# panuelosj/polystokes

Measured on AMD Instinct MI355X. Metric: Stokes-solve wall ms/step (assembly+PCG) on 256^3 grid; CG iters/sec, lower is better.
Workload: dtype f64; 1 GPU; synthetic lid-driven cavity 256x256x256, reduced tiles (tile=16, pad=2), jacobi-PCG, tol 1e-3; parallelism=1 GPU

## Files before the change

polystokes_amd/__init__.py:

```python
import ctypes as C
import os
import subprocess

import numpy as np

from . import _abi
from ._abi import (FieldsIn, FieldsOut, Params, Scene, Stats, default_params)

_HERE = os.path.dirname(os.path.abspath(__file__))
LIB_PATH = os.environ.get("PS_LIB") or os.path.join(_HERE, "libpolystokes_hip.so")
_lib = None

EXPORTED_SYMBOLS = [
    "ps_abi_version", "ps_reduced_dof", "ps_context_create", "ps_context_destroy", "ps_last_error", "ps_params_default",
    "ps_upload_fields", "ps_step_device", "ps_setup_device", "ps_solve_device", "ps_download_fields",
    "polystokes_step", "ps_apply_operator", "ps_apply_preconditioner", "ps_query_array", "ps_read_array",
    "ps_export_component_matrices", "ps_export_matrices", "ps_export_stats", "ps_bench_kernel", "ps_memory_stats", "ps_set_interrupt", "ps_solve_exported_system",
    "ps_set_slab", "ps_set_brick", "ps_comm_unique_id", "ps_comm_init_rccl", "ps_comm_selftest", "ps_comm_init_tcp", "ps_dist_stats",
    "ps_group_create", "ps_group_destroy", "ps_group_rank", "ps_group_step",
    "ps_set_warm_start", "ps_download_solution_fields", "ps_upload_density_field", "ps_set_surface_tension",
    "ps_set_solid_boundary", "ps_set_rheology", "ps_set_solve_precision",
    "ps_upload_fields_device", "ps_upload_density_field_device", "ps_download_fields_device", "ps_download_solution_fields_device",
    "ps_step_device_fields", "ps_set_velocity_extrapolation",
    "ps_upload_surface_fields", "ps_upload_surface_fields_device",
# ... 39 lines not shown
        L.ps_apply_preconditioner.argtypes = [C.c_void_p, C.c_void_p, C.c_void_p]
        L.ps_apply_preconditioner.restype = C.c_int32
        L.ps_query_array.argtypes = [C.c_void_p, C.c_char_p, C.POINTER(C.c_int32)]
        L.ps_query_array.restype = C.c_int64
        L.ps_read_array.argtypes = [C.c_void_p, C.c_char_p, C.c_void_p, C.c_int64]
        L.ps_read_array.restype = C.c_int32
        L.ps_export_component_matrices.argtypes = [C.c_void_p, C.c_char_p]
        L.ps_export_component_matrices.restype = C.c_int32
        L.ps_export_matrices.argtypes = [C.c_void_p, C.c_char_p]
        L.ps_export_matrices.restype = C.c_int32
        L.ps_export_stats.argtypes = [C.c_void_p, C.POINTER(Stats), C.c_char_p]
        L.ps_export_stats.restype = C.c_int32
        L.ps_bench_kernel.argtypes = [C.c_void_p, C.c_char_p, C.c_int32, C.POINTER(C.c_double), C.POINTER(C.c_double)]
        L.ps_bench_kernel.restype = C.c_int32
        L.ps_memory_stats.argtypes = [C.c_void_p, C.POINTER(C.c_int64)]
        L.ps_memory_stats.restype = C.c_int32
        L.ps_solve_exported_system.argtypes = [C.c_void_p, C.c_char_p, C.POINTER(Params), C.c_double, C.c_void_p, C.c_int64, C.POINTER(Stats)]
        L.ps_solve_exported_system.restype = C.c_int32
        L.ps_set_interrupt.argtypes = [C.c_void_p, C.c_void_p, C.c_void_p]
        L.ps_set_interrupt.restype = C.c_int32
        L.ps_set_slab.argtypes = [C.c_void_p, C.POINTER(_abi.SlabStruct)]
        L.ps_set_slab.restype = C.c_int32
        L.ps_set_brick.argtypes = [C.c_void_p, C.POINTER(_abi.BrickStruct)]
        L.ps_set_brick.restype = C.c_int32
        L.ps_comm_unique_id.argtypes = [C.c_void_p]
        L.ps_comm_unique_id.restype = C.c_int32
        L.ps_comm_init_rccl.argtypes = [C.c_void_p, C.c_void_p, C.c_int32, C.c_int32]
        L.ps_comm_init_rccl.restype = C.c_int32
        L.ps_comm_init_tcp.argtypes = [C.c_void_p, C.c_int32, C.c_int32, C.c_char_p, C.c_int32]
        L.ps_comm_init_tcp.restype = C.c_int32
        L.ps_comm_selftest.argtypes = [C.c_void_p]
        L.ps_comm_selftest.restype = C.c_int32
        L.ps_dist_stats.argtypes = [C.c_void_p, C.POINTER(C.c_double)]
        L.ps_dist_stats.restype = C.c_int32
        L.ps_group_create.argtypes = [C.c_int32, C.c_int32]
        L.ps_group_create.restype = C.c_void_p
        L.ps_group_destroy.argtypes = [C.c_void_p]
        L.ps_group_rank.argtypes = [C.c_void_p, C.c_int32]
        L.ps_group_rank.restype = C.c_void_p
        L.ps_group_step.argtypes = [C.c_void_p, C.POINTER(Stats)]
        L.ps_group_step.restype = C.c_int32
        L.ps_set_warm_start.argtypes = [C.c_void_p, C.c_int32]
        L.ps_set_warm_start.restype = C.c_int32
        L.ps_download_solution_fields.argtypes = [C.c_void_p, C.POINTER(_abi.SolutionOut)]
        L.ps_download_solution_fields.restype = C.c_int32
        L.ps_upload_density_field.argtypes = [C.c_void_p, C.c_void_p]
        L.ps_upload_density_field.restype = C.c_int32
        L.ps_set_surface_tension.argtypes = [C.c_void_p, C.c_double]
        L.ps_set_surface_tension.restype = C.c_int32
        L.ps_set_solid_boundary.argtypes = [C.c_void_p, C.c_int32]
        L.ps_set_solid_boundary.restype = C.c_int32
        L.ps_set_rheology.argtypes = [C.c_void_p, C.POINTER(_abi.Rheology)]
        L.ps_set_rheology.restype = C.c_int32
        L.ps_set_solve_precision.argtypes = [C.c_void_p, C.c_int32]
        L.ps_set_solve_precision.restype = C.c_int32
        L.ps_set_velocity_extrapolation.argtypes = [C.c_void_p, C.c_int32]
        L.ps_set_velocity_extrapolation.restype = C.c_int32
        L.ps_upload_fields_device.argtypes = [C.c_void_p, C.POINTER(Params), C.POINTER(FieldsIn), C.c_int32, C.c_void_p]
        L.ps_upload_fields_device.restype = C.c_int32
        L.ps_upload_density_field_device.argtypes = [C.c_void_p, C.c_void_p, C.c_int32, C.c_void_p]
        L.ps_upload_density_field_device.restype = C.c_int32
        L.ps_download_fields_device.argtypes = [C.c_void_p, C.POINTER(FieldsOut), C.c_int32, C.c_void_p]
        L.ps_download_fields_device.restype = C.c_int32
        L.ps_download_solution_fields_device.argtypes = [C.c_void_p, C.POINTER(_abi.SolutionOut), C.c_int32, C.c_void_p]
        L.ps_download_solution_fields_device.restype = C.c_int32
        L.ps_step_device_fields.argtypes = [C.c_void_p, C.POINTER(Params), C.POINTER(FieldsIn), C.POINTER(FieldsOut), C.POINTER(Stats),
                                            C.c_int32, C.c_void_p]
        L.ps_step_device_fields.restype = C.c_int32
        L.ps_upload_surface_fields.argtypes = [C.c_void_p, C.POINTER(_abi.SurfaceFields)]
        L.ps_upload_surface_fields.restype = C.c_int32
        L.ps_upload_surface_fields_device.argtypes = [C.c_void_p, C.POINTER(_abi.SurfaceFields), C.c_int32, C.c_void_p]
        L.ps_upload_surface_fields_device.restype = C.c_int32
        _lib = L
    return _lib


def device_address(a):
    if a is None:
        return None
    if isinstance(a, int):
        return a
    if hasattr(a, "ptr"):
        return int(a.ptr)
    if hasattr(a, "data_ptr"):
        return int(a.data_ptr())
    if hasattr(a, "__cuda_array_interface__"):
        return int(a.__cuda_array_interface__["data"][0])
    raise TypeError(f"no device address in {type(a).__name__}")


def stream_handle(stream):
    if stream is None:
        return None
    return int(stream) if isinstance(stream, int) else int(stream.cuda_stream)


def to_layout(a, layout):
    a = np.asarray(a, dtype=np.float32)
    return np.ascontiguousarray(a if layout == _abi.LAYOUT_X_FASTEST else a.transpose(2, 1, 0))


def from_layout(flat, shape_zyx, layout):
    flat = np.asarray(flat).ravel()
    if layout == _abi.LAYOUT_X_FASTEST:
        return flat.reshape(shape_zyx)
    return np.ascontiguousarray(flat.reshape(shape_zyx[::-1]).transpose(2, 1, 0))


class DeviceScene:

    def __init__(self, scene, layout=_abi.LAYOUT_X_FASTEST, pad=0):
        from . import _hip
        put = lambda a: _hip.DeviceBuffer.from_numpy(to_layout(a, layout), pad)
        self.layout, self.host = layout, scene
        for k in ("nx", "ny", "nz", "dx", "dt", "density", "name", "surface_tension"):
            setattr(self, k, getattr(scene, k))
        self.vel = [put(a) for a in scene.vel]
        self.collisionvel = [put(a) for a in scene.collisionvel]
        self.surface, self.collision, self.viscosity = put(scene.surface), put(scene.collision), put(scene.viscosity)
        self.weights = None if scene.weights is None else [put(a) for a in scene.weights]
        self.density_field = None if scene.density_field is None else put(scene.density_field)
        opt = lambda name: None if getattr(scene, name, None) is None else put(getattr(scene, name))
        self.surface_sigma_field, self.surface_pressure_field = opt("surface_sigma_field"), opt("surface_pressure_field")


def device_scene(scene, layout=_abi.LAYOUT_X_FASTEST, pad=0):
    return DeviceScene(scene, layout, pad)


def fields_in_device(fields):
    fi = FieldsIn()
    fi.nx, fi.ny, fi.nz = fields.nx, fields.ny, fields.nz
    fi.dx, fi.dt = fields.dx, fields.dt
    fi.orig[0] = fi.orig[1] = fi.orig[2] = 0.0
    fi.density = fields.density
    cv = getattr(fields, "collisionvel", None)
    for a in range(3):
        fi.vel[a] = device_address(fields.vel[a])
        fi.collisionvel[a] = device_address(cv[a]) if cv is not None else None
    fi.surface, fi.collision, fi.viscosity = (device_address(fields.surface), device_address(fields.collision),
                                              device_address(fields.viscosity))
    w = getattr(fields, "weights", None)
    for i in range(14):
        fi.weights[i] = device_address(w[i]) if w is not None else None
    return fi


_DT = {(1, "i"): np.int8, (4, "i"): np.int32, (4, "f"): np.float32, (8, "f"): np.float64, (4, "u"): np.uint32}


def _kind(name):
    if name.endswith(("Labels", "Indices", ".col", ".ptr", "Region", "Perm", ".chunkInfo", ".chunkRep", ".code")) or name.startswith("faceRow"):
        return "i"
    if name in ("valuesCoded", "columns16", "diagonalsCoded", "fusedStep", "streamRuns", "rowPerLane", "chebInner32", "warmStartUsed", "densityField", "launchWalk",
                "surfaceTensionReducedFaces", "surfaceFields", "solidBoundary", "solidSlipEdges", "rheologyModel", "rheologyIterations",
                "solvePrecisionUsed", "solvePassIterations",
                "velocityExtrapolation", "extrapolationLayerX", "extrapolationLayerY", "extrapolationLayerZ", "extrapolationCounts"):
        return "i"
    if name in ("ownedX", "ownedY", "ownedZ"):
        return "f"
    if False:
        return "i"
    if name == "reducedRowFace":
        return "u"
    return "f"


def process_memory_stats():
    v = (C.c_int64 * 4)()
    lib().ps_memory_stats(None, v)
    return {"live_bytes": int(v[0]), "peak_bytes": int(v[1]), "contexts": int(v[3])}


def _has_surface_fields(scene):
    return getattr(scene, "surface_sigma_field", None) is not None or getattr(scene, "surface_pressure_field", None) is not None


class PolyStokesError(RuntimeError):
    pass


class Solver:

    def __init__(self, device=0, _handle=None):
        self.L = lib()
        self._owned = _handle is None
        h = self.L.ps_context_create(device) if _handle is None else _handle
        if not h:
            raise PolyStokesError(self.L.ps_last_error(None).decode())
        self.h = C.c_void_p(h)
        self.stats = Stats()
        self.scene = None

    def close(self):
        if getattr(self, "h", None):
            if self._owned:
                self.L.ps_context_destroy(self.h)
            self.h = None

    def set_interrupt(self, fn):
        if fn is None:
            self._cb = None
            self._check(self.L.ps_set_interrupt(self.h, None, None))
            return
        self._cb = C.CFUNCTYPE(C.c_int32, C.c_void_p)(lambda user: 1 if fn() else 0)
        self._check(self.L.ps_set_interrupt(self.h, C.cast(self._cb, C.c_void_p), None))

    def set_warm_start(self, mode):
        self._check(self.L.ps_set_warm_start(self.h, int(mode)))

    def set_surface_tension(self, sigma):
        return self._check(self.L.ps_set_surface_tension(self.h, float(sigma)), allow=(1, -2))

    def set_solid_boundary(self, mode):
        return self._check(self.L.ps_set_solid_boundary(self.h, int(mode)), allow=(1, -2))

    def set_rheology(self, model=_abi.RHEOLOGY_HERSCHEL_BULKLEY, flow_index=1.0, yield_stress=0.0, min_shear_rate=1e-3,
                     min_viscosity=1e-3, max_viscosity=1e6, passes=0):
        r = _abi.Rheology(int(model), int(passes), float(flow_index), float(yield_stress), float(min_shear_rate), float(min_viscosity),
                          float(max_viscosity))
        return self._check(self.L.ps_set_rheology(self.h, C.byref(r)), allow=(1, -2))

    def set_solve_precision(self, mode):
        return self._check(self.L.ps_set_solve_precision(self.h, int(mode)), allow=(1, -2))

    def set_velocity_extrapolation(self, layers):
        return self._check(self.L.ps_set_velocity_extrapolation(self.h, int(layers)), allow=(1, -2))

    def solution_fields(self):
        sh = _abi.grid_shapes(self.scene.nx, self.scene.ny, self.scene.nz)
        out = {name: np.empty(sh[grid], np.float32) for name, grid in _abi.SOLUTION_FIELDS}
        so = _abi.SolutionOut()
        so.pressure = out["pressure"].ctypes.data
        for a, name in enumerate(("txx", "tyy", "tzz")):
            so.tauDiag[a] = out[name].ctypes.data
        for a, name in enumerate(("tyz", "txz", "txy")):
            so.tauEdge[a] = out[name].ctypes.data
        self._check(self.L.ps_download_solution_fields(self.h, C.byref(so)))
        return out

    def set_slab(self, slab):
        st = _abi.SlabStruct(slab.rank, slab.world, slab.zLoOwned, slab.zHiOwned, slab.hasLower, slab.hasUpper, slab.z0)
        self._check(self.L.ps_set_slab(self.h, C.byref(st)))

    def set_brick(self, b):
        i3 = C.c_int32 * 3
        st = _abi.BrickStruct(b.rank, b.world, i3(*b.dims), i3(*b.lo), i3(*b.hi), i3(*b.hasLower), i3(*b.hasUpper), i3(*b.g0))
        self._check(self.L.ps_set_brick(self.h, C.byref(st)))

    def comm_selftest(self):
        self._check(self.L.ps_comm_selftest(self.h))

    def dist_stats(self):
        v = (C.c_double * 8)()
        self._check(self.L.ps_dist_stats(self.h, v))
        return {"halo_bytes_per_iter": v[0], "owned_dofs": v[1], "overlap": bool(v[2]),
                "exchange_ms_per_transport": (v[3] / v[4]) if v[4] else None, "exchange_samples": int(v[4]),
                "allreduce_ms": (v[5] / v[6]) if v[6] else None, "allreduce_samples": int(v[6]), "halo_label_changes": int(v[7])}

    def memory_stats(self):
        v = (C.c_int64 * 4)()
        self.L.ps_memory_stats(self.h, v)
        return {"live_bytes": int(v[0]), "peak_bytes": int(v[1]), "deferred_bytes": int(v[2]), "contexts": int(v[3])}

    def comm_init(self, uid_bytes, rank, world):
        buf = C.create_string_buffer(bytes(uid_bytes), 128)
        self._check(self.L.ps_comm_init_rccl(self.h, buf, rank, world))

    def comm_init_tcp(self, rank, world, host="127.0.0.1", base_port=29600):
        self._check(self.L.ps_comm_init_tcp(self.h, rank, world, host.encode(), base_port))

    def __del__(self):
        try:
            self.close()
        except Exception:
            pass

    def _check(self, rc, allow=(1,)):
        if rc == _abi.FAILED or rc not in allow:
            raise PolyStokesError(f"rc={rc}: {self.L.ps_last_error(self.h).decode()}")
        return rc

    def upload(self, scene, params):
        self.scene, self.params = scene, params
        fi = scene.fields_in()
        self._check(self.L.ps_upload_fields(self.h, C.byref(params), C.byref(fi)))
        self._scene_surface_tension(scene)
        if getattr(scene, "density_field", None) is not None:
            self._check(self.upload_density_field(scene.density_field))
        if _has_surface_fields(scene):
            self._check(self.upload_surface_fields(scene.surface_sigma_field, scene.surface_pressure_field))

    def _scene_surface_tension(self, scene):
        sigma = getattr(scene, "surface_tension", None)
        if sigma is not None:
            self._check(self.L.ps_set_surface_tension(self.h, float(sigma)))

    def upload_density_field(self, field):
        if field is None:
            return self._check(self.L.ps_upload_density_field(self.h, None), allow=(1, -2))
        sh = _abi.grid_shapes(self.scene.nx, self.scene.ny, self.scene.nz)["center"] if self.scene is not None else None
        f = np.ascontiguousarray(field, dtype=np.float32)
        if sh is not None and f.shape != sh:
            f = f.reshape(sh)
        self._density_keep = f
        return self._check(self.L.ps_upload_density_field(self.h, f.ctypes.data), allow=(1, -2))

# ... 284 lines not shown
```

polystokes_amd/csrc/ps_blocks.hip:

```cpp
#include "ps_context.hpp"
#include "ps_setup_util.hpp"

using namespace ps;

namespace {

constexpr int BS = SETUP_BS;

struct BlockArgs {
    Grid g;
    double invDx;
    const float* lw[7];
    const float* fw[7];
    const int32_t* lab[7];
    const int32_t* act[7];
    const int32_t* reg[7];
    const int32_t* sys[7];
    const int32_t* sysT[3];
    const int32_t* faceRow[3];
    const float* vel[3];
    const float* cvel[3];
    CellField visc;
    FaceDensity dens;
    int64_t nP, nA, faceOff[3];
// ... 378 lines not shown
        cnt[j] = n;
        if (slipEdge(A, ea, c)) atomicAdd(A.slipEdges, 1);
        return;
    }
    sortRows4(rows, vals);
    const int p0 = ptr[j];
#pragma unroll
    for (int k = 0; k < 4; ++k)
        if (k < n) { col[p0 + k] = rows[k]; if (val) val[p0 + k] = vals[k]; code[p0 + k] = encodeVal(A, vals[k]); }
    rhsPT[j] = rhs;
    const double vw = clampd((double)A.fw[4 + ea][c], 0.1, 1.0) * (double)A.lw[4 + ea][c];
    const float ox = ea == 0 ? 0.5f : 0.f, oy = ea == 1 ? 0.5f : 0.f, oz = ea == 2 ? 0.5f : 0.f;
    const double visc = (double)A.visc.sample(A.g, (float)q.x + ox, (float)q.y + oy, (float)q.z + oz);
    const double invVisc = clampd(1. / visc, 0., 1e10);
    uInv[t] = A.own.sample(4 + ea, q.x, q.y, q.z) ? 2. * invVisc * vw : 0.;
    if (uDiag) uDiag[t] = 0.5 * visc * clampd(1. / vw, 0., 1.e2);
}

BlockArgs makeArgs(ps_context* c) {
    BlockArgs A;
    A.g = c->g; A.invDx = c->invDx;
    for (int s = 0; s < 7; ++s) {
        A.lw[s] = c->liquidW[s].p; A.fw[s] = c->fluidW[s].p;
        A.lab[s] = c->labels[s].p; A.act[s] = c->activeIdx[s].p; A.reg[s] = c->reducedIdx[s].p; A.sys[s] = c->sysIdx[s].p;
    }
    for (int a = 0; a < 3; ++a) { A.faceRow[a] = c->faceRow[a].p; A.vel[a] = c->vel[a].p; A.cvel[a] = c->cvel[a].p; A.sysT[a] = c->sysIdxT[a].p; }
    A.visc = c->viscSource(); A.dens = c->densSource();
    A.nP = c->nPressures; A.nA = c->nActiveVs;
    A.faceOff[0] = 0; A.faceOff[1] = c->nFace[0]; A.faceOff[2] = c->nFace[0] + c->nFace[1];
    A.own = c->own();
    A.valScale = c->valScale;
    A.codeFail = c->counters.p + CTR_CODE_FAIL;
    A.regionOwned = (c->slabEnabled && c->regionCount > 0) ? c->regionOwned.p : nullptr;
    A.freeSlip = c->solidBoundaryUsed == PS_SOLID_FREE_SLIP ? 1 : 0;
    A.slipEdges = A.freeSlip ? c->slipEdges.p : nullptr;
    return A;
}

__global__ void k_chunk_len4(const int32_t* __restrict__ ptr, const int2* __restrict__ chunkRows, int nChunks, int32_t* __restrict__ len4, int32_t* __restrict__ maxLen) {
    const int ch = blockIdx.x * blockDim.x + threadIdx.x;
    if (ch > nChunks) return;
    int n = 0;
    if (ch < nChunks) { const int2 cr = chunkRows[ch]; n = ptr[cr.x + cr.y] - ptr[cr.x]; atomicMax(maxLen, n); }
    len4[ch] = (n + 3) & ~3;
}
__global__ void __launch_bounds__(BS) k_col16_build(const int32_t* __restrict__ ptr, const int32_t* __restrict__ col, const int8_t* __restrict__ code,
                                                    const int2* __restrict__ chunkRows, const int32_t* __restrict__ start4, uint16_t* __restrict__ col16,
                                                    int8_t* __restrict__ code4, int32_t* __restrict__ winBase, int4* __restrict__ chunkInfo,
                                                    uint8_t* __restrict__ len8, int32_t* __restrict__ fail, int32_t* __restrict__ chunkRep, int nChunks) {
    const int lane = threadIdx.x & 63;
    const int chunk = blockIdx.x * (BS / 64) + (int)(threadIdx.x >> 6);
    if (chunk >= nChunks) return;
    if (lane == 0) chunkRep[chunk] = chunk;
    const int2 cr = chunkRows[chunk];
    const int r0 = cr.x;
    const int p0 = ptr[r0], p1 = ptr[r0 + cr.y];
    const int q0 = start4[chunk], q1 = start4[chunk + 1];
    if (lane == 0) chunkInfo[chunk] = make_int4(q0, (p1 - p0) | (cr.y << 16), cr.x, cr.x);
    for (int i = lane; i < cr.y; i += 64) len8[r0 + i] = (uint8_t)(ptr[r0 + i + 1] - ptr[r0 + i]);
    constexpr int SL = 32;
    if (p1 - p0 > SL * 64) { if (lane == 0) *fail = 1; return; }
    int c[SL];
    unsigned open = 0u;
#pragma unroll
    for (int u = 0; u < SL; ++u) {
        const int i = lane + u * 64;
        const bool o = p0 + i < p1;
        c[u] = o ? col[p0 + i] : 0x7fffffff;
        if (o) open |= 1u << u;
        if (q0 + i < q1) { code4[q0 + i] = o ? code[p0 + i] : (int8_t)0; if (!o) col16[q0 + i] = 0; }
    }
    int used = 16;
    for (int w = 0; w < 16; ++w) {
        int m = 0x7fffffff;
#pragma unroll
        for (int u = 0; u < SL; ++u) if ((open >> u) & 1u) m = min(m, c[u]);
        for (int o = 32; o > 0; o >>= 1) m = min(m, __shfl_xor(m, o));
        const int base = m;
        if (base == 0x7fffffff) { used = w; break; }
        if (lane == 0) winBase[(int64_t)chunk * 16 + w] = base;
#pragma unroll
        for (int u = 0; u < SL; ++u)
            if (((open >> u) & 1u) && c[u] - base < 4096) {
                col16[q0 + lane + u * 64] = (uint16_t)((w << 12) | (c[u] - base));
                open &= ~(1u << u);
            }
    }
    if (lane == 0) for (int w = used; w < 16; ++w) winBase[(int64_t)chunk * 16 + w] = 0;
    if (open) *fail = 1;
}
__global__ void __launch_bounds__(64) k_chunk_hash(const int4* __restrict__ chunkInfo, const uint16_t* __restrict__ col16, const int8_t* __restrict__ code4,
                                                   const uint8_t* __restrict__ len8, unsigned long long* __restrict__ hash, int weak) {
    const int chunk = blockIdx.x;
    const int4 ci = chunkInfo[chunk];
    const int n4 = ((ci.y & 0xffff) + 3) & ~3, rows = (int)((unsigned)ci.y >> 16);
    unsigned long long h = 0;
    if (!weak)
    for (int i = threadIdx.x; i < n4; i += 64)
        h += mix64(((unsigned long long)i << 32) | ((unsigned long long)col16[ci.x + i] << 8) | (uint8_t)code4[ci.x + i]);
    if (!weak)
    for (int i = threadIdx.x; i < rows; i += 64) h += mix64(0x4000000000000000ull | ((unsigned long long)i << 32) | len8[ci.z + i]);
    for (int o = 32; o > 0; o >>= 1) h += __shfl_down(h, o, 64);
    if (threadIdx.x == 0) {
        h = mix64(h ^ (((unsigned long long)(unsigned)n4 << 32) | (unsigned)rows));
        hash[chunk] = h == HASH_EMPTY ? 0ull : h;
    }
}
__global__ void k_chunk_rep_insert(const unsigned long long* __restrict__ hash, int nChunks, unsigned long long* __restrict__ keys, int32_t* __restrict__ vals, unsigned mask) {
    const int chunk = blockIdx.x * blockDim.x + threadIdx.x;
    if (chunk >= nChunks) return;
    const unsigned long long h = hash[chunk];
    hashInsertMin(keys, vals, mask, (unsigned)(h >> 17) & mask, h, chunk);
}
__global__ void __launch_bounds__(64) k_chunk_share(const unsigned long long* __restrict__ hash, const unsigned long long* __restrict__ keys, const int32_t* __restrict__ vals,
                                                    unsigned mask, int4* __restrict__ chunkInfo, const uint16_t* __restrict__ col16, const int8_t* __restrict__ code4,
                                                    const uint8_t* __restrict__ len8, const uint8_t* __restrict__ rowCode, int codeRows,
                                                    unsigned long long* __restrict__ uniqueLen, int32_t* __restrict__ chunkRep) {
    const int chunk = blockIdx.x;
    const unsigned long long h = hash[chunk];
    unsigned slot = (unsigned)(h >> 17) & mask;
    while (keys[slot] != h) slot = (slot + 1) & mask;
    const int rep = vals[slot];
    const int4 ci = chunkInfo[chunk];
    const int n = ci.y & 0xffff, n4 = (n + 3) & ~3, rows = (int)((unsigned)ci.y >> 16);
    bool same = rep != chunk;
    if (same) {
        const int4 cr = chunkInfo[rep];
        same = cr.y == ci.y;
        if (same) {
            for (int i = threadIdx.x; i < n4; i += 64) same = same && col16[ci.x + i] == col16[cr.x + i] && code4[ci.x + i] == code4[cr.x + i];
            for (int i = threadIdx.x; i < rows; i += 64) {
                same = same && len8[ci.z + i] == len8[cr.z + i];
                if (rowCode) {
                    const bool a = ci.z + i < codeRows, b = cr.z + i < codeRows;
                    same = same && a == b && (!a || rowCode[ci.z + i] == rowCode[cr.z + i]);
                }
            }
        }
        same = __all(same) != 0;
        if (same && threadIdx.x == 0) { chunkInfo[chunk].x = cr.x; chunkInfo[chunk].w = cr.z; chunkRep[chunk] = rep; }
    }
    if (!same && threadIdx.x == 0) atomicAdd(uniqueLen, (unsigned long long)n4);
}
__global__ void __launch_bounds__(BS) k_val4_build(const int32_t* __restrict__ ptr, const double* __restrict__ val,
                                                   const int4* __restrict__ chunkInfo, double* __restrict__ val4) {
    const int chunk = blockIdx.x;
    const int4 ci = chunkInfo[chunk];
    const int p0 = ptr[ci.z], n = ci.y & 0xffff, q0 = ci.x;
    const int n4 = (n + 3) & ~3;
    for (int i = threadIdx.x; i < n4; i += BS) val4[q0 + i] = i < n ? val[p0 + i] : 0.;
}
__device__ inline int ellCodeWidth(int W) { return W > 4 ? 8 : (W > 0 ? 4 : 0); }
constexpr int32_t ELL_NULL_BASE = 0x1ffff000;
__global__ void __launch_bounds__(BS) k_ell_plan(const int4* __restrict__ chunkInfo, const uint8_t* __restrict__ len8, const int32_t* __restrict__ chunkRep,
                                                 int32_t* __restrict__ colLen, int32_t* __restrict__ codeLen, int32_t* __restrict__ wpack, int32_t* __restrict__ fail) {
    __shared__ int wmax[BS / 64];
    const int chunk = blockIdx.x;
    const int4 ci = chunkInfo[chunk];
    const int rows = (int)((unsigned)ci.y >> 16);
    int len = (int)threadIdx.x < rows ? (int)len8[ci.z + threadIdx.x] : 0;
    for (int o = 32; o > 0; o >>= 1) len = max(len, __shfl_down(len, o, 64));
    if ((threadIdx.x & 63) == 0) wmax[threadIdx.x >> 6] = len;
    __syncthreads();
    if (threadIdx.x == 0) {
        int cl = 0, vl = 0, wp = 0;
        for (int u = 0; u < BS / 64; ++u) {
            const int W = (wmax[u] + 1) & ~1;
            if (W > 8) *fail = 1;
            cl += 64 * W; vl += 64 * ellCodeWidth(W); wp |= (W & 15) << (4 * u);
        }
        const bool own = chunkRep[chunk] == chunk;
        colLen[chunk] = own ? cl : 0; codeLen[chunk] = own ? vl : 0; wpack[chunk] = wp;
    }
}
__global__ void __launch_bounds__(BS) k_ell_fill(const int4* __restrict__ chunkInfo, const uint8_t* __restrict__ len8, const int32_t* __restrict__ chunkRep,
                                                 const uint16_t* __restrict__ col16, const int8_t* __restrict__ code4, const int32_t* __restrict__ colBegin,
                                                 const int32_t* __restrict__ codeBegin, const int32_t* __restrict__ wpack, uint16_t* __restrict__ ecol,
                                                 int8_t* __restrict__ ecode, int4* __restrict__ echunk, int32_t* __restrict__ winBase) {
    const int chunk = blockIdx.x;
    const int rep = chunkRep[chunk];
    const bool nullOk = winBase[chunk * 16 + 15] == 0 || winBase[chunk * 16 + 15] == ELL_NULL_BASE;
    __syncthreads();
    if (nullOk && threadIdx.x == 0) winBase[chunk * 16 + 15] = ELL_NULL_BASE;
    const int4 ci = chunkInfo[chunk];
    const int rows = (int)((unsigned)ci.y >> 16);
    const int wp = wpack[chunk];
    if (threadIdx.x == 0) echunk[chunk] = make_int4(colBegin[rep], codeBegin[rep], ci.z, rows | (wp << 12));
    if (rep != chunk) return;
    const int len = (int)len8[ci.z + min((int)threadIdx.x, rows - 1)];
    int total;
    const int mine = (int)threadIdx.x < rows ? len : 0;
    const int e0 = blockExclusiveScan(mine, &total);
    __shared__ int lastE0;
    if ((int)threadIdx.x == rows - 1) lastE0 = e0;
    __syncthreads();
    const int eb = ci.x + ((int)threadIdx.x < rows ? e0 : lastE0);
    const int u = threadIdx.x >> 6, lane = threadIdx.x & 63;
    const int W = (wp >> (4 * u)) & 15, CW = ellCodeWidth(W);
    if (W == 0 || u * 64 >= rows) return;
    int pre = 0, preC = 0;
    for (int v = 0; v < u; ++v) { const int w = (wp >> (4 * v)) & 15; pre += w; preC += ellCodeWidth(w); }
    uint16_t* oc = ecol + (size_t)colBegin[chunk] + (size_t)64 * pre + (size_t)lane * W;
    int8_t* ov = ecode + (size_t)codeBegin[chunk] + (size_t)64 * preC + (size_t)lane * CW;
    uint16_t lastc = 0;
    for (int k = 0; k < W; ++k) {
        if (k < len) lastc = col16[eb + k];
        oc[k] = (k < len || !nullOk) ? lastc : (uint16_t)0xf000;
    }
    for (int k = 0; k < CW; ++k) ov[k] = k < len ? code4[eb + k] : (int8_t)0;
}
}
void ps_context::buildEll(ps::DevCSR& M) {
    M.ellok = false;
    static const bool off = envInt(PS_ENV("PS_NO_ELL"), 0) != 0 ||
                            envInt(PS_ENV("PS_PIPE_GRID"), 1) == 0;
    if (off || !M.col16ok || !M.packed || M.nChunks == 0 || (uint64_t)std::max(M.rows, M.cols) * 8 >= 0xffff8000ull) return;
    const int nChunks = M.nChunks;
    DevBuf<int32_t>& colBegin = scrEllCol; DevBuf<int32_t>& codeBegin = scrEllCode; DevBuf<int32_t>& wpack = scrEllW;
    colBegin.alloc((size_t)nChunks + 1); codeBegin.alloc((size_t)nChunks + 1); wpack.alloc((size_t)nChunks);
    HIP_CHECK(hipMemsetAsync(colBegin.p + nChunks, 0, sizeof(int32_t), stream));
    HIP_CHECK(hipMemsetAsync(codeBegin.p + nChunks, 0, sizeof(int32_t), stream));
    HIP_CHECK(hipMemsetAsync(counters.p + CTR_ELL_TOO_LONG, 0, sizeof(int32_t), stream));
    hipLaunchKernelGGL(k_ell_plan, dim3((unsigned)nChunks), dim3(BS), 0, stream, (const int4*)M.chunkInfo.p, (const uint8_t*)M.len8.p, (const int32_t*)M.chunkRep.p,
                       colBegin.p, codeBegin.p, wpack.p, counters.p + CTR_ELL_TOO_LONG);
    scanBlock.alloc((size_t)gridFor(nChunks + 1, PS_SCAN_TILE) + 16);
    (void)exclusiveScanI32(colBegin.p, nChunks + 1, CTR_ELL_COLS);
    (void)exclusiveScanI32(codeBegin.p, nChunks + 1, CTR_ELL_CODES);
    int32_t w[3];
    fetchCounters(CTR_ELL_TOO_LONG, 3, w);
    const int32_t tooLong = w[0];
    const int64_t totCol = w[1], totCode = w[2];
    if (totCol < 0 || totCode < 0 || (uint64_t)totCol * 2 >= 0xffffffffull || tooLong != 0) return;
    M.ellCols = totCol; M.ellCodes = totCode; M.ellUniqueCols = totCol;
    M.ecol.alloc((size_t)totCol + 64); M.ecode.alloc((size_t)totCode + 64); M.echunk.alloc((size_t)nChunks);
    hipLaunchKernelGGL(k_ell_fill, dim3((unsigned)nChunks), dim3(BS), 0, stream, (const int4*)M.chunkInfo.p, (const uint8_t*)M.len8.p, (const int32_t*)M.chunkRep.p,
                       (const uint16_t*)M.col16.p, (const int8_t*)M.code4.p, (const int32_t*)colBegin.p, (const int32_t*)codeBegin.p, (const int32_t*)wpack.p,
                       M.ecol.p, M.ecode.p, M.echunk.p, M.winBase.p);
    M.ellok = true;
    if (PS_ENV_VERBOSE()) std::fprintf(stderr, "[polystokes] row-per-lane stream: %d chunks, %lld column slots and %lld code bytes in the distinct runs (nnz %lld)\n",
                                           nChunks, (long long)totCol, (long long)totCode, (long long)M.nnz);
}
namespace {
__global__ void k_decode_values(const int8_t* __restrict__ code, double scale, int64_t n, double* __restrict__ val) {
    for (int64_t i = (int64_t)blockIdx.x * blockDim.x + threadIdx.x; i < n; i += (int64_t)gridDim.x * blockDim.x) val[i] = (double)code[i] * scale;
}
}
void ps_context::ensureValues(ps::DevCSR& M) {
    if (M.val.p || M.nnz == 0) return;
    if (!M.packed || !M.code.p) throw Error("internal: a block without values and without codes");
    M.val.alloc((size_t)M.nnz);
    hipLaunchKernelGGL(k_decode_values, dim3(2048), dim3(BS), 0, stream, (const int8_t*)M.code.p, valScale, M.nnz, M.val.p);
}
void ps_context::buildVal4(ps::DevCSR& M) {
    if (!M.col16ok || M.val4.p) return;
    ensureValues(M);
    M.val4.alloc((size_t)M.streamLen + 8);
    hipLaunchKernelGGL(k_val4_build, dim3((unsigned)M.nChunks), dim3(BS), 0, stream, M.ptr.p, M.val.p, M.chunkInfo.p, M.val4.p);
}
void ps_context::buildCol16(ps::DevCSR& M, Counter slot, const std::vector<int32_t>& cuts, const uint8_t* rowCode, int codeRows) {
    M.col16ok = false;
    M.ellok = false;
    M.nChunks = 0;
    M.val4.free();
    const char* e = PS_ENV("PS_COL32");
    if (M.rows == 0 || M.nnz == 0 || (e && atoi(e) != 0)) return;
    std::vector<int2> rowsOf;
    {
        constexpr int CHUNK_ALIGN_MIN = 512;
        static const bool plain = envInt(PS_ENV("PS_CHUNK_PLAIN"), 0) != 0;
        bool ok = !plain && cuts.size() >= 2 && cuts.front() == 0 && (int64_t)cuts.back() == M.rows;
        for (size_t i = 1; ok && i < cuts.size(); ++i) ok = cuts[i] >= cuts[i - 1];
        auto emit = [&](int64_t lo, int64_t hi) { for (int64_t r = lo; r < hi; r += BS) rowsOf.push_back(make_int2((int)r, (int)std::min<int64_t>(BS, hi - r))); };
        if (!ok) emit(0, M.rows);
        else {
            int64_t runLo = 0;
            for (size_t i = 0; i + 1 < cuts.size(); ++i) {
                const int64_t lo = cuts[i], hi = cuts[i + 1];
                if (hi - lo >= CHUNK_ALIGN_MIN) { emit(runLo, lo); emit(lo, hi); runLo = hi; }
            }
            emit(runLo, M.rows);
        }
    }
    const int nChunks = (int)rowsOf.size();
    DevBuf<int2>& chunkRows = scrChunkRows;
    chunkRows.alloc((size_t)nChunks);
    HIP_CHECK(hipMemcpyAsync(chunkRows.p, rowsOf.data(), (size_t)nChunks * sizeof(int2), hipMemcpyHostToDevice, stream));
    DevBuf<int32_t>& start4 = scrStart4;
    start4.alloc((size_t)nChunks + 1);
    HIP_CHECK(hipMemsetAsync(counters.p + CTR_CHUNK_MAX, 0, sizeof(int32_t), stream));
    hipLaunchKernelGGL(k_chunk_len4, dim3(gridFor(nChunks + 1, BS)), dim3(BS), 0, stream, M.ptr.p, (const int2*)chunkRows.p, nChunks, start4.p, counters.p + CTR_CHUNK_MAX);
    const int64_t total4 = exclusiveScanI32(start4.p, nChunks + 1);
    if (total4 < 0) return;
    const int maxLen = readCounter(CTR_CHUNK_MAX);
    M.nv = std::max(1, (maxLen + 4 * BS - 1) / (4 * BS));
    if (M.nv > 2) return;
    if ((uint64_t)std::max(M.rows, M.cols) * 8 >= 0xffffffffull || (uint64_t)total4 * 2 >= 0xffffffffull) return;
    M.streamLen = total4;
    M.uniqueLen = total4;
    M.nChunks = nChunks;
    M.col16.alloc((size_t)total4 + 8); M.code4.alloc((size_t)total4 + 8);
    M.winBase.alloc((size_t)nChunks * 16); M.chunkInfo.alloc((size_t)nChunks); M.len8.alloc((size_t)M.rows); M.chunkRep.alloc((size_t)nChunks);
    HIP_CHECK(hipMemsetAsync(counters.p + slot, 0, sizeof(int32_t), stream));
    hipLaunchKernelGGL(k_col16_build, dim3((unsigned)((nChunks + BS / 64 - 1) / (BS / 64))), dim3(BS), 0, stream, M.ptr.p, M.col.p, M.code.p, (const int2*)chunkRows.p, start4.p, M.col16.p,
                       M.code4.p, M.winBase.p, M.chunkInfo.p, M.len8.p, counters.p + slot, M.chunkRep.p, nChunks);
    M.col16ok = readCounter(slot) == 0;
    if (M.col16ok && !M.packed) buildVal4(M);
    static const bool noShare = envInt(PS_ENV("PS_NO_SHARED_RUNS"), 0) != 0;
    static const bool weakHash = envInt(PS_ENV("PS_WEAK_CHUNK_HASH"), 0) != 0;
    if (M.col16ok && M.packed && shareRuns && !noShare && nChunks > 1) {
        unsigned cap = 1024;
        while (cap < 4u * (unsigned)nChunks) cap <<= 1;
        DevBuf<unsigned long long>& hash = scrHash; DevBuf<unsigned long long>& keys = scrKeys; DevBuf<unsigned long long>& uniq = scrUniq;
        DevBuf<int32_t>& vals = scrVals;
        hash.alloc((size_t)nChunks); keys.alloc(cap); vals.alloc(cap); uniq.alloc(1);
        HIP_CHECK(hipMemsetAsync(keys.p, 0xff, (size_t)cap * 8, stream));
        HIP_CHECK(hipMemsetAsync(vals.p, 0x7f, (size_t)cap * 4, stream));
        HIP_CHECK(hipMemsetAsync(uniq.p, 0, 8, stream));
        hipLaunchKernelGGL(k_chunk_hash, dim3((unsigned)nChunks), dim3(64), 0, stream, (const int4*)M.chunkInfo.p, (const uint16_t*)M.col16.p, (const int8_t*)M.code4.p,
                           (const uint8_t*)M.len8.p, hash.p, weakHash ? 1 : 0);
        hipLaunchKernelGGL(k_chunk_rep_insert, dim3(gridFor(nChunks, BS)), dim3(BS), 0, stream, (const unsigned long long*)hash.p, nChunks, keys.p, vals.p, cap - 1);
        hipLaunchKernelGGL(k_chunk_share, dim3((unsigned)nChunks), dim3(64), 0, stream, (const unsigned long long*)hash.p, (const unsigned long long*)keys.p,
                           (const int32_t*)vals.p, cap - 1, M.chunkInfo.p, (const uint16_t*)M.col16.p, (const int8_t*)M.code4.p, (const uint8_t*)M.len8.p, rowCode, codeRows, uniq.p, M.chunkRep.p);
        unsigned long long u = 0;
        HIP_CHECK(hipMemcpyAsync(&u, uniq.p, 8, hipMemcpyDeviceToHost, stream));
        HIP_CHECK(hipStreamSynchronize(stream));
        M.uniqueLen = (int64_t)u;
    }
    if (PS_ENV_VERBOSE()) std::fprintf(stderr, "[polystokes] compressed stream: rows %lld nnz %lld, %d chunks, fullest %d (nv %d), ok %d, distinct runs hold %lld of %lld entries\n",
                                           (long long)M.rows, (long long)M.nnz, nChunks, maxLen, M.nv, (int)M.col16ok, (long long)M.uniqueLen, (long long)M.streamLen);
}

namespace {
constexpr unsigned long long DICT_EMPTY = 0xfff8dead0000beefull;
__device__ inline int dictHash(unsigned long long k) { k ^= k >> 33; k *= 0xff51afd7ed558ccdull; k ^= k >> 29; return (int)(k & 255ull); }
__global__ void __launch_bounds__(BS) k_dict_build(const double* __restrict__ v, int64_t n, unsigned long long* __restrict__ table, int32_t* __restrict__ overflow) {
    __shared__ unsigned long long snap[256];
    snap[threadIdx.x] = __hip_atomic_load(&table[threadIdx.x], __ATOMIC_RELAXED, __HIP_MEMORY_SCOPE_AGENT);
    __syncthreads();
    const int64_t stride = (int64_t)gridDim.x * blockDim.x;
    const int64_t rounds = (n + stride - 1) / stride;
    for (int64_t k = 0; k < rounds; ++k) {
        const int64_t i = k * stride + (int64_t)blockIdx.x * blockDim.x + threadIdx.x;
        const bool have = i < n;
        const unsigned long long key = have ? (unsigned long long)__double_as_longlong(v[i]) : 0ull;
        bool miss = have;
        if (have && key == DICT_EMPTY) { *overflow = 1; miss = false; }
        if (miss) {
            const int h0 = dictHash(key);
            for (int probe = 0; probe < 256; ++probe) {
                const unsigned long long cur = snap[(h0 + probe) & 255];
                if (cur == key) { miss = false; break; }
                if (cur == DICT_EMPTY) break;
            }
        }
        unsigned long long m = __ballot(miss);
        if (m != 0ull && __hip_atomic_load(overflow, __ATOMIC_RELAXED, __HIP_MEMORY_SCOPE_AGENT) != 0) return;
        while (m != 0ull) {
            const int leader = __ffsll((long long)m) - 1;
            const unsigned long long lk = ((unsigned long long)(unsigned)__shfl((int)(key >> 32), leader, 64) << 32) | (unsigned)__shfl((int)(key & 0xffffffffull), leader, 64);
            if ((int)(threadIdx.x & 63) == leader) {
                int h = dictHash(lk);
                bool placed = false;
                for (int probe = 0; probe < 256 && !placed; ++probe) {
                    unsigned long long cur = __hip_atomic_load(&table[h], __ATOMIC_RELAXED, __HIP_MEMORY_SCOPE_AGENT);
                    if (cur == DICT_EMPTY) cur = atomicCAS(&table[h], DICT_EMPTY, lk), cur = (cur == DICT_EMPTY) ? lk : cur;
                    if (cur == lk) { placed = true; snap[h] = lk; }
                    else h = (h + 1) & 255;
                }
                if (!placed) *overflow = 1;
            }
            if (miss && key == lk) miss = false;
            m = __ballot(miss);
        }
    }
}
__global__ void k_dict_code(const double* __restrict__ v, int64_t n, const unsigned long long* __restrict__ table, uint8_t* __restrict__ code) {
    for (int64_t i = (int64_t)blockIdx.x * blockDim.x + threadIdx.x; i < n; i += (int64_t)gridDim.x * blockDim.x) {
        const unsigned long long key = (unsigned long long)__double_as_longlong(v[i]);
        int h = dictHash(key);
        for (int probe = 0; probe < 256 && table[h] != key; ++probe) h = (h + 1) & 255;
        code[i] = (uint8_t)h;
    }
}
__global__ void k_dict_init(unsigned long long* table) { table[threadIdx.x] = DICT_EMPTY; }
__global__ void k_dict_finish(unsigned long long* table) { if (table[threadIdx.x] == DICT_EMPTY) table[threadIdx.x] = 0ull; }
}
void ps_context::buildDiagonalCodes() {
    uCoded = mcCoded = false;
    const char* e = PS_ENV("PS_NO_DIAG_CODES");
    if (e && atoi(e) != 0) return;
    auto build = [&](const DevBuf<double>& vals, int64_t n, DevBuf<uint8_t>& code, DevBuf<double>& dict) -> bool {
        if (n <= 0) return false;
        dict.alloc(256); code.alloc((size_t)n);
// ... 180 lines not shown
```

polystokes_amd/csrc/ps_context.hip:

```cpp
#include <algorithm>
#include <chrono>
#include <cstdio>
#include <cstring>
#include <ctime>
#include <fstream>

#include "ps_context.hpp"
#include "ps_setup_util.hpp"

using namespace ps;

namespace {

struct StageTimer {
    hipEvent_t ev[PS_STAGE_COUNT + 1];
    hipStream_t s;
    int n = 0;
    explicit StageTimer(hipStream_t st) : s(st) {
        for (auto& e : ev) HIP_CHECK(hipEventCreate(&e));
    }
    ~StageTimer() { for (auto& e : ev) (void)hipEventDestroy(e); }
    void mark(int i) { HIP_CHECK(hipEventRecord(ev[i], s)); }
    double ms(int a, int b) { float f = 0; HIP_CHECK(hipEventElapsedTime(&f, ev[a], ev[b])); return f; }
};
// ... 236 lines not shown
    T.mark(7);
    constructPreconditioner();
    T.mark(8);
    HIP_CHECK(hipStreamSynchronize(stream));
    const auto w1 = std::chrono::high_resolution_clock::now();
    std::memset(&lastStats, 0, sizeof(lastStats));
    lastStats.result = PS_INCOMPLETE;
    fillDimData(&lastStats);
    lastStats.solveData[0] = -1; lastStats.solveData[1] = -1; lastStats.solveData[2] = -1; lastStats.solveData[3] = -1;
    lastStats.solveData[4] = 1000.0 * (double)(std::clock() - Z.c0) / CLOCKS_PER_SEC;
    lastStats.solveData[5] = std::chrono::duration<double, std::milli>(w1 - Z.w0).count();
    lastStats.stage_ms[PS_STAGE_WEIGHTS] = T.ms(0, 1);
    lastStats.stage_ms[PS_STAGE_CLASSIFY] = T.ms(1, 2);
    lastStats.stage_ms[PS_STAGE_REGIONS] = T.ms(2, 3);
    lastStats.stage_ms[PS_STAGE_INDICES] = T.ms(3, 4);
    lastStats.stage_ms[PS_STAGE_TILE_MATRICES] = T.ms(4, 5);
    lastStats.stage_ms[PS_STAGE_BLOCKS] = T.ms(5, 6);
    lastStats.stage_ms[PS_STAGE_ASSEMBLE] = T.ms(6, 7);
    lastStats.stage_ms[PS_STAGE_PRECOND] = T.ms(7, 8);
    setupState.reset();
    setupPhaseDone = 2;
    isSetup = true; isSolved = false;
    registerArrays();
}

int ps_context::solveStage(ps_stats* stats) {
    if (!isSetup) throw Error("ps_setup_device has not been called");
    HIP_CHECK(hipSetDevice(device));
    StageTimer T(stream);
    int result = PS_INCOMPLETE;
    extrapUsedHost = 0;
    const std::clock_t c0 = std::clock();
    const auto w0 = std::chrono::high_resolution_clock::now();
    T.mark(0);
    if (P.doSolve) {
        result = solve();
        HIP_CHECK(hipStreamSynchronize(stream));
        const auto w1 = std::chrono::high_resolution_clock::now();
        lastStats.solveData[0] = solveError;
        lastStats.solveData[1] = solveIterations;
        lastStats.solveData[2] = 1000.0 * (double)(std::clock() - c0) / CLOCKS_PER_SEC;
        lastStats.solveData[3] = std::chrono::duration<double, std::milli>(w1 - w0).count();
    }
    T.mark(1);
    buildValidFaces();
    const bool apply = result != PS_UNSUPPORTED_SOLVER && !(P.doSolve && interrupted) && (result == PS_SUCCESS || P.keepNonConvergedResults);
    if (apply) {
        recoverVelocityFromPressureStress();
        T.mark(2);
        applySolutionToVelocity();
        if (extrapSet > 0 && !slabEnabled) extrapolateVelocity(extrapSet);
        if ((warmMode == PS_WARM_PREVIOUS_STEP || rheoCarry) && P.doSolve && P.solverType == PS_PCG_MATRIX_VECTOR_PRODUCTS && !slabEnabled) carryWarmStart();
    } else {
        T.mark(2);
        for (int a = 0; a < 3; ++a)
            HIP_CHECK(hipMemcpyAsync(velOut[a].p, vel[a].p, (size_t)g.count(1 + a) * sizeof(float), hipMemcpyDeviceToDevice, stream));
    }
    T.mark(3);
    HIP_CHECK(hipStreamSynchronize(stream));
    lastStats.stage_ms[PS_STAGE_SOLVE] = T.ms(0, 1);
    lastStats.stage_ms[PS_STAGE_RECOVER] = T.ms(1, 2);
    lastStats.stage_ms[PS_STAGE_WRITEBACK] = T.ms(2, 3);
    lastStats.result = result;
    lastStats.usedBiCGStab = usedBiCGStab;
    if (rheoModelUsed != PS_RHEOLOGY_NEWTONIAN && P.doSolve) rheoIters.push_back(solveIterations);
    isSolved = true;
    registerArrays();
    if (stats) *stats = lastStats;
    return result;
}

void ps_context::registerArrays() {
    arrays.clear();
    auto reg = [&](const std::string& n, const void* p, int64_t c, int e) { arrays[n] = ArrayInfo{p, c, e}; };
    auto regHost = [&](const std::string& n, const void* p, int64_t c, int e) { reg(n, p, c, e); arrays[n].host = true; };
    for (int s = 0; s < 7; ++s) {
        const int64_t n = g.count(s);
        reg(std::string(kSampleName[s]) + "LiquidWeights", liquidW[s].p, n, 4);
        reg(std::string(kSampleName[s]) + "FluidWeights", fluidW[s].p, n, 4);
        reg(std::string(kSampleName[s]) + "Labels", labels[s].p, n, 4);
        reg(std::string(kSampleName[s]) + "ActiveIndices", activeIdx[s].p, n, 4);
        reg(std::string(kSampleName[s]) + "ReducedIndices", reducedIdx[s].p, n, 4);
    }
    const int64_t R = regionCount;
    reg("reducedRegionCOM", COM.p, R * 3, 8);
    reg("reducedRegionCenterOfMass", COM.p, R * 3, 8);
    reg("reducedRegionBestFitVectors", cfit.p, R * PS_RD, 8);
    reg("reducedMassMatrices", Mr.p, R * PS_RD * PS_RD, 8);
    reg("reducedViscosityMatrices", Kv.p, R * PS_RD * PS_RD, 8);
    reg("Inv_Mr_plus_2JDtuDJ", Binv.p, R * PS_RD * PS_RD, 8);
    reg("reducedRHSVector", rhsR.p, R * PS_RD, 8);
    auto regp = [&](const std::string& n, const void* p, int64_t c, const int32_t* perm, int64_t off) {
        ArrayInfo a{p, c, 8};
        a.perm = perm; a.permOffset = off;
        arrays[n] = a;
    };
    regp("McInv", McInv.p, nActiveVs, permRow.p, 0);
    regp("activeRHSVector", rhsA.p, nActiveVs, permRow.p, 0);
    regp("oldActiveVs", oldVs.p, nActiveVs, permRow.p, 0);
    regp("uInv", uInv.p, nStresses, permSys.p, nPressures);
    if (P.exportComponentMatrices) {
        regp("Mc", Mc.p, nActiveVs, permRow.p, 0);
        regp("u", uDiag.p, nStresses, permSys.p, nPressures);
    }
    regp("pressureRHSVector", rhsPT.p, nPressures, permSys.p, 0);
    regp("stressRHSVector", rhsPT.p, nStresses, permSys.p, nPressures);
    regp("b", b.p, nSystem, permSys.p, 0);
    regp("solutionVector", x.p, nSystem, permSys.p, 0);
    regp("guessVector", guess.p, nSystem, permSys.p, 0);
    if (warmX0Valid) regp("warmStartVector", warmX0.p, nSystem, permSys.p, 0);
    regHost("warmStartUsed", &warmUsedHost, 1, 4);
    regHost("solvePrecisionUsed", &solvePrecisionUsedHost, 1, 4);
    if (solvePrecisionUsedHost != 0) {
        regHost("solvePassIterations", passIters.data(), (int64_t)passIters.size(), 4);
        regHost("solveTrueResidual", &trueResidualHost, 1, 8);
    }
    densFieldHost = densField ? 1 : 0;
    regHost("densityField", &densFieldHost, 1, 4);
    regHost("surfaceTension", &sigmaUsed, 1, 8);
    regHost("surfaceFields", &surfFieldsUsed, 1, 4);
    if (sigmaUsed != 0. || (surfFieldsUsed & 1)) reg("surfaceCurvature", kappaC.p, g.count(0), 4);
    if (sigmaUsed != 0. || surfFieldsUsed != 0) reg("surfaceTensionReducedFaces", stReduced.p, 1, 4);
    if (surfFieldsUsed != 0 && surfQ.p) reg("surfaceGhostPressure", surfQ.p, g.count(0), 8);
    regHost("solidBoundary", &solidBoundaryUsed, 1, 4);
    if (solidBoundaryUsed == PS_SOLID_FREE_SLIP) reg("solidSlipEdges", slipEdges.p, 1, 4);
    regHost("rheologyModel", &rheoModelUsed, 1, 4);
    if (rheoModelUsed != PS_RHEOLOGY_NEWTONIAN) {
        reg("rheologyStrainRate", rheoRate.p, g.count(0), 4);
        reg("rheologyViscosity", rheoMu.p, g.count(0), 4);
        regHost("rheologyIterations", rheoIters.data(), (int64_t)rheoIters.size(), 4);
    }
    regHost("velocityExtrapolation", &extrapUsedHost, 1, 4);
    if (extrapUsedHost > 0) {
        static const char* axn[3] = {"X", "Y", "Z"};
        for (int a = 0; a < 3; ++a) reg(std::string("extrapolationLayer") + axn[a], extrapLayer[a].p, g.count(1 + a), 1);
        reg("extrapolationCounts", extrapCounts.p, extrapUsedHost, 4);
    }
    if (P.preconditioner == PS_PRE_DIAGONAL) regp("dinv", dinv.p, nSystem, permSys.p, 0);
    if (isSolved) {
        regp("recoveredActiveVelocity", recovered.p, nActiveVs, permRow.p, 0);
        reg("recoveredReducedVelocity", recovered.p ? recovered.p + nActiveVs : nullptr, nReducedVs, 8);
    }
    regHost("valuesCoded", &valuesCodedHost, 1, 4);
    diagFlagsHost = (uCoded ? 1 : 0) | (mcCoded ? 2 : 0);
    regHost("diagonalsCoded", &diagFlagsHost, 1, 4);
    regHost("columns16", &columns16Host, 1, 4);
    regHost("fusedStep", &fusedStepHost, 1, 4);
    regHost("launchWalk", launchWalkHost, 5 * LAUNCH_WALK_FIELDS, 4);
    chebInner32Host = chebInner32 ? 1 : 0;
    regHost("chebInner32", &chebInner32Host, 1, 4);
    streamRunsHost[0] = S.col16ok ? (int32_t)S.uniqueLen : 0; streamRunsHost[1] = S.col16ok ? (int32_t)S.streamLen : 0;
    streamRunsHost[2] = St.col16ok ? (int32_t)St.uniqueLen : 0; streamRunsHost[3] = St.col16ok ? (int32_t)St.streamLen : 0;
    regHost("streamRuns", streamRunsHost, 4, 4);
    rowPerLaneHost[0] = ((S.ellok && S.packed) ? 1 : 0) | ((St.ellok && St.packed) ? 2 : 0); rowPerLaneHost[1] = ilPlaneMajor;
    regHost("rowPerLane", rowPerLaneHost, 2, 4);
    reg("sysPerm", permSys.p, nSystem, 4);
    reg("rowPerm", permRow.p, nActiveVs, 4);
    reg("S.ptr", S.ptr.p, S.rows + 1, 4); reg("S.col", S.col.p, S.nnz, 4); reg("S.val", S.val.p, S.nnz, 8);
    reg("St.ptr", St.ptr.p, St.rows + 1, 4); reg("St.col", St.col.p, St.nnz, 4); reg("St.val", St.val.p, St.nnz, 8);
    if (S.col16ok) { reg("S.chunkInfo", S.chunkInfo.p, (int64_t)S.nChunks * 4, 4); reg("S.chunkRep", S.chunkRep.p, S.nChunks, 4); }
    if (St.col16ok) { reg("St.chunkInfo", St.chunkInfo.p, (int64_t)St.nChunks * 4, 4); reg("St.chunkRep", St.chunkRep.p, St.nChunks, 4); }
    if (S.packed) reg("S.code", S.code.p, S.nnz, 1);
    if (St.packed) reg("St.code", St.code.p, St.nnz, 1);
    reg("reducedRowFace", rrowFace.p, nReducedRows, 4);
    reg("reducedRowRegion", rrowRegion.p, nReducedRows, 4);
    static const char* ax[3] = {"X", "Y", "Z"};
    for (int a = 0; a < 3; ++a) {
        reg(std::string("vel") + ax[a], velOut[a].p, g.count(1 + a), 4);
        reg(std::string("valid") + ax[a], valid[a].p, g.count(1 + a), 4);
        reg(std::string("faceRow") + ax[a], faceRow[a].p, g.count(1 + a), 4);
        if (slabEnabled && isSolved) reg(std::string("owned") + ax[a], ownedFace[a].p, g.count(1 + a), 4);
    }
}

#define PS_TRY(ctx, ...)                                                     \
    ps::SinkScope sinkScope_((ctx) ? &(ctx)->deferred : nullptr);            \
    try { __VA_ARGS__ } catch (const ps::Error& e) {                         \
        if (ctx) { (ctx)->err = e.msg; (ctx)->drainDeferred(false); }        \
        return PS_FAILED;                                                    \
    } catch (const std::exception& e) {                                      \
        if (ctx) { (ctx)->err = e.what(); (ctx)->drainDeferred(false); }     \
        return PS_FAILED;                                                    \
    }

static std::string g_createError;

static bool writeMarketVector(const std::string& fn, const std::vector<double>& v) {
    std::ofstream out(fn.c_str(), std::ios::out);
    if (!out) return false;
    out.flags(std::ios_base::scientific);
    out.precision(17);
    out << "%%MatrixMarket matrix array real general\n";
    out << v.size() << " " << 1 << "\n";
    for (double d : v) out << d << "\n";
    return true;
}
static bool writeMarketSparse(const std::string& fn, int64_t rows, int64_t cols, const std::vector<int64_t>& ptr,
                              const std::vector<int32_t>& col, const std::vector<double>& val) {
    std::ofstream out(fn.c_str(), std::ios::out);
    if (!out) return false;
    out.flags(std::ios_base::scientific);
    out.precision(17);
    out << "%%MatrixMarket matrix coordinate  real general" << std::endl;
    out << rows << " " << cols << " " << val.size() << "\n";
    for (int64_t r = 0; r < rows; ++r)
        for (int64_t p = ptr[(size_t)r]; p < ptr[(size_t)r + 1]; ++p) out << r + 1 << " " << col[(size_t)p] + 1 << " " << val[(size_t)p] << "\n";
    return true;
}
template <class T>
static std::vector<T> fetch(ps_context* c, const T* dptr, int64_t n) {
    std::vector<T> h((size_t)std::max<int64_t>(n, 0));
    if (n > 0) {
        HIP_CHECK(hipMemcpyAsync(h.data(), dptr, (size_t)n * sizeof(T), hipMemcpyDeviceToHost, c->stream));
        HIP_CHECK(hipStreamSynchronize(c->stream));
    }
    return h;
}

void ps_context::buildExplicitA(std::vector<int64_t>& aptr, std::vector<int32_t>& acol, std::vector<double>& aval) {
    const int64_t n = nSystem, nA = nActiveVs, nP = nPressures;
    auto sp = fetch(this, S.ptr.p, nRows + 1);
    auto sc = fetch(this, S.col.p, S.nnz);
    ensureValues(S);
    auto sv = fetch(this, S.val.p, S.nnz);
    auto mc = fetch(this, McInv.p, nA);
    auto ui = fetch(this, uInv.p, n);
    auto perm = fetch(this, permSys.p, n);
    std::vector<int32_t> inv((size_t)n);
    for (int64_t i = 0; i < n; ++i) inv[(size_t)perm[(size_t)i]] = (int32_t)i;
    struct T { int32_t r, c; double v; };
    std::vector<T> t;
    double est = 0;
    for (int64_t f = 0; f < nA; ++f) { const double l = (double)(sp[(size_t)f + 1] - sp[(size_t)f]); est += l * l; }
    std::vector<std::vector<int32_t>> regCols((size_t)regionCount);
    std::vector<int32_t> rreg;
    std::vector<uint32_t> rface;
    if (regionCount > 0) {
        rreg = fetch(this, rrowRegion.p, nReducedRows);
        rface = fetch(this, rrowFace.p, nReducedRows);
        for (int64_t q = 0; q < nReducedRows; ++q)
            for (int32_t p = sp[(size_t)(nA + q)]; p < sp[(size_t)(nA + q) + 1]; ++p) regCols[(size_t)rreg[(size_t)q]].push_back(sc[(size_t)p]);
        for (auto& v : regCols) { std::sort(v.begin(), v.end()); v.erase(std::unique(v.begin(), v.end()), v.end()); est += (double)v.size() * (double)v.size(); }
    }
    if (est > 4.0e8) throw Error("the explicit matrix A is too large to export (its reduced part is dense per tile): export the component matrices instead");
    t.reserve((size_t)est + (size_t)n);
    for (int64_t f = 0; f < nA; ++f) {
        const double d = -dt * mc[(size_t)f];
        for (int32_t a = sp[(size_t)f]; a < sp[(size_t)f + 1]; ++a)
            for (int32_t b2 = sp[(size_t)f]; b2 < sp[(size_t)f + 1]; ++b2)
                t.push_back({inv[(size_t)sc[(size_t)a]], inv[(size_t)sc[(size_t)b2]], d * sv[(size_t)a] * sv[(size_t)b2]});
    }
    if (regionCount > 0) {
        auto com = fetch(this, COM.p, regionCount * 3);
        auto bi = fetch(this, Binv.p, regionCount * PS_RD * PS_RD);
        std::vector<int64_t> first((size_t)regionCount + 1, 0);
        for (int64_t q = 0; q < nReducedRows; ++q) first[(size_t)rreg[(size_t)q] + 1]++;
        for (int64_t r = 0; r < regionCount; ++r) first[(size_t)r + 1] += first[(size_t)r];
        for (int64_t r = 0; r < regionCount; ++r) {
            const std::vector<int32_t>& cols = regCols[(size_t)r];
            const size_t m = cols.size();
            if (m == 0) continue;
            std::vector<double> JS((size_t)PS_RD * m, 0.), W((size_t)PS_RD * m, 0.);
            for (int64_t q = first[(size_t)r]; q < first[(size_t)r + 1]; ++q) {
                int i, j, k, axis;
                unpackFace(rface[(size_t)q], i, j, k, axis);
                double o[3], cf[PS_RD];
                faceOffset(&com[(size_t)r * 3], dx, make_int3(gOff[0], gOff[1], gOff[2]), axis, i, j, k, o);
                basisRow(o[0], o[1], o[2], axis, cf);
                for (int32_t p = sp[(size_t)(nA + q)]; p < sp[(size_t)(nA + q) + 1]; ++p) {
                    const size_t lc = (size_t)(std::lower_bound(cols.begin(), cols.end(), sc[(size_t)p]) - cols.begin());
                    for (int e = 0; e < PS_RD; ++e) JS[(size_t)e * m + lc] += cf[e] * sv[(size_t)p];
                }
            }
            for (int e = 0; e < PS_RD; ++e)
                for (int g2 = 0; g2 < PS_RD; ++g2) {
                    const double bv = bi[(size_t)r * PS_RD * PS_RD + (size_t)e * PS_RD + g2];
                    if (bv == 0.) continue;
                    for (size_t c2 = 0; c2 < m; ++c2) W[(size_t)e * m + c2] += bv * JS[(size_t)g2 * m + c2];
                }
            for (size_t a = 0; a < m; ++a)
                for (size_t b2 = 0; b2 < m; ++b2) {
                    double s2 = 0;
                    for (int e = 0; e < PS_RD; ++e) s2 += JS[(size_t)e * m + a] * W[(size_t)e * m + b2];
                    t.push_back({inv[(size_t)cols[a]], inv[(size_t)cols[b2]], -s2});
                }
        }
    }
    for (int64_t i = nP; i < n; ++i) t.push_back({(int32_t)i, (int32_t)i, -0.5 * ui[(size_t)perm[(size_t)i]]});
    std::stable_sort(t.begin(), t.end(), [](const T& a, const T& b2) { return a.r != b2.r ? a.r < b2.r : a.c < b2.c; });
    aptr.assign((size_t)n + 1, 0); acol.clear(); aval.clear();
    size_t p = 0;
    for (int64_t r = 0; r < n; ++r) {
        aptr[(size_t)r] = (int64_t)aval.size();
        while (p < t.size() && t[p].r == r) {
            const int32_t cc = t[p].c;
            double s2 = 0;
            while (p < t.size() && t[p].r == r && t[p].c == cc) { s2 += t[p].v; ++p; }
            acol.push_back(cc); aval.push_back(s2);
        }
    }
    aptr[(size_t)n] = (int64_t)aval.size();
}

extern "C" {

int32_t ps_abi_version(void) { return 1; }
// ... 261 lines not shown

int32_t ps_upload_fields_device(ps_context* c, const ps_params* p, const ps_fields_in* in, int32_t layout, void* stream) {
    if (!c) return PS_FAILED;
    PS_TRY(c, {
        HIP_CHECK(hipSetDevice(c->device));
        const std::string why = c->refuseFieldsIn(in, layout);
        if (!why.empty()) { c->err = "ps_upload_fields_device: " + why; return PS_INVALID; }
        c->upload(p, in, layout, (hipStream_t)stream);
        return PS_SUCCESS;
    })
}
int32_t ps_upload_density_field_device(ps_context* c, const float* density, int32_t layout, void* stream) {
    if (!c) return PS_FAILED;
    PS_TRY(c, {
        if (!c->uploaded) { c->err = "ps_upload_density_field: call ps_upload_fields first"; return PS_INVALID; }
        HIP_CHECK(hipSetDevice(c->device));
        std::string why;
        if (const char* m = ps_context::layoutRefusal(layout)) why = m;
        else if (density) why = c->checkDeviceField(density, c->g.count(0), "density");
        if (!why.empty()) { c->err = "ps_upload_density_field_device: " + why; return PS_INVALID; }
        why = c->uploadDensityDevice(density, layout, (hipStream_t)stream);
        if (!why.empty()) { c->err = why; return PS_INVALID; }
        return PS_SUCCESS;
    })
}
int32_t ps_upload_surface_fields_device(ps_context* c, const ps_surface_fields* f, int32_t layout, void* stream) {
    if (!c) return PS_FAILED;
    PS_TRY(c, {
        if (!c->uploaded) { c->err = "ps_upload_surface_fields: call ps_upload_fields first"; return PS_INVALID; }
        HIP_CHECK(hipSetDevice(c->device));
        std::string why;
        if (const char* m = ps_context::layoutRefusal(layout)) why = m;
        if (why.empty() && f && f->sigma) why = c->checkDeviceField(f->sigma, c->g.count(0), "sigma");
        if (why.empty() && f && f->pressure) why = c->checkDeviceField(f->pressure, c->g.count(0), "pressure");
        if (!why.empty()) {
            HIP_CHECK(hipStreamSynchronize(c->stream));
            c->dropSurfaceFields();
            c->drainDeferred(true);
            c->err = "ps_upload_surface_fields_device: " + why;
            return PS_INVALID;
        }
        why = c->uploadSurfaceFields(f, true, layout, (hipStream_t)stream);
        if (!why.empty()) { c->err = "ps_upload_surface_fields: " + why; return PS_INVALID; }
        return PS_SUCCESS;
    })
}
int32_t ps_download_fields_device(ps_context* c, const ps_fields_out* out, int32_t layout, void* stream) {
    if (!c || !out) return PS_FAILED;
    PS_TRY(c, {
        if (!c->uploaded) throw Error("ps_upload_fields has not been called");
        HIP_CHECK(hipSetDevice(c->device));
        std::string why;
        if (const char* m = ps_context::layoutRefusal(layout)) why = m;
        for (int a = 0; a < 3 && why.empty(); ++a) {
            if (out->vel[a]) why = c->checkDeviceField(out->vel[a], c->g.count(1 + a), "out vel");
            if (why.empty() && out->valid[a]) why = c->checkDeviceField(out->valid[a], c->g.count(1 + a), "out valid");
        }
        if (!why.empty()) { c->err = "ps_download_fields_device: " + why; return PS_INVALID; }
        c->downloadDevice(out, layout, (hipStream_t)stream);
        return PS_SUCCESS;
    })
}
int32_t ps_download_solution_fields_device(ps_context* c, const ps_solution_out* out, int32_t layout, void* stream) {
    if (!c || !out) return PS_FAILED;
    PS_TRY(c, {
        if (c->slabEnabled) throw Error("ps_download_solution_fields is a single-domain call");
        if (!c->isSetup || !c->isSolved) throw Error("ps_download_solution_fields: no solve since the last setup");
        HIP_CHECK(hipSetDevice(c->device));
        const float* dst[7] = {out->pressure, out->tauDiag[0], out->tauDiag[1], out->tauDiag[2], out->tauEdge[0], out->tauEdge[1], out->tauEdge[2]};
        std::string why;
        if (const char* m = ps_context::layoutRefusal(layout)) why = m;
        for (int q = 0; q < 7 && why.empty(); ++q) if (dst[q]) why = c->checkDeviceField(dst[q], c->solutionGridCount(q), "solution grid");
        if (!why.empty()) { c->err = "ps_download_solution_fields_device: " + why; return PS_INVALID; }
        c->downloadSolutionDevice(out, layout, (hipStream_t)stream);
        return PS_SUCCESS;
    })
}
int32_t ps_step_device_fields(ps_context* c, const ps_params* p, const ps_fields_in* in, const ps_fields_out* out, ps_stats* st, int32_t layout,
                              void* stream) {
    if (!c) return PS_FAILED;
    PS_TRY(c, {
        HIP_CHECK(hipSetDevice(c->device));
        std::string why = c->refuseFieldsIn(in, layout);
        if (why.empty() && out && in && in->nx > 0 && in->ny > 0 && in->nz > 0 && in->nx <= 1022 && in->ny <= 1022 && in->nz <= 1022) {
            const ps::Grid gg{in->nx, in->ny, in->nz, 0};
            for (int a = 0; a < 3 && why.empty(); ++a) {
                if (out->vel[a]) why = c->checkDeviceField(out->vel[a], gg.count(1 + a), "out vel");
                if (why.empty() && out->valid[a]) why = c->checkDeviceField(out->valid[a], gg.count(1 + a), "out valid");
            }
        }
        if (!why.empty()) { c->err = "ps_step_device_fields: " + why; return PS_INVALID; }
        c->upload(p, in, layout, (hipStream_t)stream);
        const int result = c->stepWithPasses(st);
        c->drainDeferred(true);
        if (out) c->downloadDevice(out, layout, (hipStream_t)stream);
        if (p->exportMatrices && p->exportDataPrefix) ps_export_matrices(c, p->exportDataPrefix);
        if (p->exportComponentMatrices && p->exportDataPrefix) ps_export_component_matrices(c, p->exportDataPrefix);
        if (p->exportStats && p->exportDataPrefix) ps_export_stats(c, st, p->exportDataPrefix);
        return result;
    })
}

int32_t ps_apply_operator(ps_context* c, const double* x, double* y) {
    if (!c) return PS_FAILED;
    PS_TRY(c, {
        if (!c->isSetup) throw Error("not set up");
        HIP_CHECK(hipSetDevice(c->device));
        const size_t n = (size_t)c->nSystem;
        c->tmp1.alloc(n); c->tmp2.alloc(n);
        c->tmp3.alloc(n);
        HIP_CHECK(hipMemcpyAsync(c->tmp3.p, x, n * sizeof(double), hipMemcpyHostToDevice, c->stream));
        hipLaunchKernelGGL(k_scatter_perm8, dim3(gridFor((int64_t)n, 256)), dim3(256), 0, c->stream, c->tmp1.p, c->tmp3.p, c->permSys.p, (int64_t)n);
        c->applyOperator(c->tmp1.p, c->tmp2.p, c->dotPartials.p);
        hipLaunchKernelGGL(k_gather_perm8, dim3(gridFor((int64_t)n, 256)), dim3(256), 0, c->stream, c->tmp3.p, c->tmp2.p, c->permSys.p, (int64_t)0, (int64_t)n);
        HIP_CHECK(hipMemcpyAsync(y, c->tmp3.p, n * sizeof(double), hipMemcpyDeviceToHost, c->stream));
        HIP_CHECK(hipStreamSynchronize(c->stream));
        return PS_SUCCESS;
    })
}

int32_t ps_apply_preconditioner(ps_context* c, const double* rin, double* zout) {
    if (!c || !rin || !zout) return PS_FAILED;
    PS_TRY(c, {
        if (!c->isSetup) throw Error("not set up");
        if (c->slabEnabled) throw Error("ps_apply_preconditioner is a single-domain call");
        HIP_CHECK(hipSetDevice(c->device));
        const size_t n = (size_t)c->nSystem;
        c->tmp3.alloc(n); c->tmp4.alloc(n); c->tmp1.alloc(n); c->tmp2.alloc(n);
        HIP_CHECK(hipMemcpyAsync(c->tmp3.p, rin, n * sizeof(double), hipMemcpyHostToDevice, c->stream));
        hipLaunchKernelGGL(k_scatter_perm8, dim3(gridFor((int64_t)n, 256)), dim3(256), 0, c->stream, c->tmp4.p, c->tmp3.p, c->permSys.p, (int64_t)n);
        c->applyPreconditionerDevice(c->tmp4.p, c->tmp1.p, c->tmp2.p);
        hipLaunchKernelGGL(k_gather_perm8, dim3(gridFor((int64_t)n, 256)), dim3(256), 0, c->stream, c->tmp3.p, c->tmp1.p, c->permSys.p, (int64_t)0, (int64_t)n);
        HIP_CHECK(hipMemcpyAsync(zout, c->tmp3.p, n * sizeof(double), hipMemcpyDeviceToHost, c->stream));
        HIP_CHECK(hipStreamSynchronize(c->stream));
        return PS_SUCCESS;
    })
}

int64_t ps_query_array(ps_context* c, const char* name, int32_t* elem_bytes) {
    if (!c || !name) return -1;
    auto it = c->arrays.find(name);
    if (it == c->arrays.end()) return -1;
    if (elem_bytes) *elem_bytes = it->second.elem;
    return it->second.count;
}
int32_t ps_read_array(ps_context* c, const char* name, void* dst, int64_t dst_bytes) {
    if (!c || !name) return PS_FAILED;
    PS_TRY(c, {
        if (c->isSetup && (std::strcmp(name, "S.val") == 0 || std::strcmp(name, "St.val") == 0)) {
            ps::DevCSR& M = name[1] == '.' ? c->S : c->St;
            c->ensureValues(M);
            c->arrays[name].dptr = M.val.p;
        }
        auto it = c->arrays.find(name);
        if (it == c->arrays.end()) throw Error(std::string("unknown array ") + name);
        const int64_t need = it->second.count * it->second.elem;
        if (dst_bytes < need) throw Error("destination too small");
        if (need > 0 && it->second.host) {
            std::memcpy(dst, it->second.dptr, (size_t)need);
        } else if (need > 0) {
            HIP_CHECK(hipSetDevice(c->device));
            const void* src = it->second.dptr;
            if (it->second.perm) {
                const int64_t n = it->second.count;
                c->tmp3.alloc((size_t)n);
                hipLaunchKernelGGL(k_gather_perm8, dim3(gridFor(n, 256)), dim3(256), 0, c->stream, c->tmp3.p, (const double*)it->second.dptr,
                                   it->second.perm, it->second.permOffset, n);
                src = c->tmp3.p;
            }
            HIP_CHECK(hipMemcpyAsync(dst, src, (size_t)need, hipMemcpyDeviceToHost, c->stream));
            HIP_CHECK(hipStreamSynchronize(c->stream));
        }
        return PS_SUCCESS;
    })
}

int32_t ps_bench_kernel(ps_context* c, const char* kernel, int32_t iters, double* avg_ms, double* algorithmic_bytes) {
    if (!c || !kernel) return PS_FAILED;
    PS_TRY(c, {
        if (!c->isSetup) throw Error("not set up");
        HIP_CHECK(hipSetDevice(c->device));
        std::string k(kernel);
        const bool seq = k.compare(0, 4, "seq:") == 0;
        if (seq) k = k.substr(4);
        const bool unshared = k.size() > 5 && k.compare(k.size() - 5, 5, "_fp64") == 0 && c->S.col16ok && c->St.col16ok && c->S.packed;
        struct Reshare { ps_context* c; bool on; ~Reshare() { if (on) { try { c->buildStreams(true); } catch (...) {} } } } reshare{c, unshared};
        if (unshared) c->buildStreams(false);
        std::vector<std::string> pred;
        if (seq) {
            if (k == "spmv_St" || k == "spmv_St_r") pred = {"spmv_S", "tiles"};
            else if (k == "cg_update_xp_u") pred = {"spmv_St_r"};
            else if (k == "spmv_S") pred = {"cg_update_xp"};
            else if (k == "tiles") pred = {"spmv_S"};
            else if (k == "cg_update_r") pred = {"spmv_St"};
            else if (k == "cg_update_xp") pred = {"cg_update_r"};
            else throw Error("seq: unknown kernel " + k);
        }
        hipEvent_t e0, e1;
        HIP_CHECK(hipEventCreate(&e0)); HIP_CHECK(hipEventCreate(&e1));
        const size_t n = (size_t)c->nSystem;
        c->tmp1.alloc(n); c->tmp2.alloc(n);
        HIP_CHECK(hipMemcpyAsync(c->tmp1.p, c->b.p, n * sizeof(double), hipMemcpyDeviceToDevice, c->stream));
        for (int w = 0; w < 3; ++w) { for (const std::string& q : pred) ps_bench_launch(c, q, c->tmp1.p, c->tmp2.p); ps_bench_launch(c, k, c->tmp1.p, c->tmp2.p); }
        float ms = 0;
        if (!seq) {
            HIP_CHECK(hipEventRecord(e0, c->stream));
            for (int i = 0; i < iters; ++i) ps_bench_launch(c, k, c->tmp1.p, c->tmp2.p);
            HIP_CHECK(hipEventRecord(e1, c->stream));
            HIP_CHECK(hipEventSynchronize(e1));
            HIP_CHECK(hipEventElapsedTime(&ms, e0, e1));
        } else {
            for (int i = 0; i < iters; ++i) {
                for (const std::string& q : pred) ps_bench_launch(c, q, c->tmp1.p, c->tmp2.p);
                HIP_CHECK(hipEventRecord(e0, c->stream));
                ps_bench_launch(c, k, c->tmp1.p, c->tmp2.p);
                HIP_CHECK(hipEventRecord(e1, c->stream));
                HIP_CHECK(hipEventSynchronize(e1));
                float one = 0;
                HIP_CHECK(hipEventElapsedTime(&one, e0, e1));
                ms += one;
            }
        }
        (void)hipEventDestroy(e0); (void)hipEventDestroy(e1);
        if (avg_ms) *avg_ms = (double)ms / (double)iters;
        if (algorithmic_bytes) {
            const double nnz = (double)c->S.nnz, rowsS = (double)c->nRows, rowsT = (double)c->nSystem;
            auto endsWith = [&](const char* suf) { const size_t m = std::strlen(suf); return k.size() > m && k.compare(k.size() - m, m, suf) == 0; };
            const bool fp64 = endsWith("_fp64"), csr = endsWith("_csr");
            const std::string kb = fp64 ? k.substr(0, k.size() - 5) : (csr ? k.substr(0, k.size() - 4) : k);
            auto perNnz = [&](const ps::DevCSR& M) { return csr ? 12. : (M.col16ok ? ((M.packed && !fp64) ? 3. : 10.) : (M.packed ? 5. : 12.)); };
            auto c16 = [&](const ps::DevCSR& M) { return !csr && M.col16ok; };
            const double perNnzS = perNnz(c->S), perNnzT = perNnz(c->St);
            const double entS = nnz, entT = nnz;
            const double winS = c16(c->S) ? 80. * (double)c->S.nChunks : 0., winT = c16(c->St) ? 80. * (double)c->St.nChunks : 0.;
            auto ell = [&](const ps::DevCSR& M) { return c16(M) && M.packed && M.ellok && !fp64; };
            const double ptrS = c16(c->S) ? (ell(c->S) ? 0. : 1.) : 4., ptrT = c16(c->St) ? (ell(c->St) ? 0. : 1.) : 4.;
            const double dMc = (c16(c->S) && c->mcCoded) ? 1. : 8., dU = (c16(c->St) && c->uCoded) ? 1. : 8.;
            const double bS = winS + perNnzS * entS + ptrS * (rowsS + 1) + 8. * rowsS + 8. * rowsT + dMc * (double)c->nActiveVs;
            const double bT = winT + perNnzT * entT + ptrT * (rowsT + 1) + 8. * rowsT + 8. * rowsS + 8. * rowsT + dU * rowsT;
            const double dg = c->P.preconditioner == PS_PRE_DIAGONAL ? (double)sizeof(ps::diag_t) : 0.;
            if (kb == "spmv_S") *algorithmic_bytes = bS;
            else if (kb == "spmv_St") *algorithmic_bytes = bT;
            else if (kb == "spmv_St_r") *algorithmic_bytes = bT + (8. + dg) * rowsT;
            else if (kb == "cg_update_xp_u") *algorithmic_bytes = (40. + dg + (c->uCoded ? 1. : 8.)) * rowsT;
            else if (kb == "apply") *algorithmic_bytes = bS + bT + (double)c->nReducedRows * (8. + 4. + 8. + 8. + 4.);
            else if (kb == "tiles") *algorithmic_bytes = (double)c->nReducedRows * (8. + 4. + 8. + 4.);
            else if (kb == "cg_update_r") *algorithmic_bytes = (24. + dg) * rowsT;
            else if (kb == "cg_update_xp") *algorithmic_bytes = (40. + dg) * rowsT;
            else if (kb == "cg_update_xr") *algorithmic_bytes = (c->P.preconditioner == PS_PRE_DIAGONAL ? 56. : 48.) * rowsT;
            else if (kb == "cg_update_p") *algorithmic_bytes = (c->P.preconditioner == PS_PRE_DIAGONAL ? 32. : 24.) * rowsT;
            else *algorithmic_bytes = 0;
        }
        return PS_SUCCESS;
    })
}

int32_t ps_export_stats(ps_context* c, const ps_stats* st, const char* prefix) {
    if (!c || !st || !prefix) return PS_FAILED;
    PS_TRY(c, {
        std::vector<double> dd(st->dimData, st->dimData + 27), sd(st->solveData, st->solveData + 6);
        if (!writeMarketVector(std::string(prefix) + "dimData.mtx", dd)) throw Error("cannot write dimData.mtx");
        if (!writeMarketVector(std::string(prefix) + "solveData.mtx", sd)) throw Error("cannot write solveData.mtx");
        return PS_SUCCESS;
    })
}

int32_t ps_export_component_matrices(ps_context* c, const char* prefix) {
    if (!c || !prefix) return PS_FAILED;
    PS_TRY(c, {
        if (!c->isSetup) throw Error("not set up");
        HIP_CHECK(hipSetDevice(c->device));
        const std::string pre(prefix);
        const int64_t nA = c->nActiveVs, nP = c->nPressures, nT = c->nStresses, R = c->regionCount;
        auto sp = fetch(c, c->S.ptr.p, c->S.rows + 1);
        auto sc = fetch(c, c->S.col.p, c->S.nnz);
        c->ensureValues(c->S);
        auto sv = fetch(c, c->S.val.p, c->S.nnz);
        auto rface = fetch(c, c->rrowFace.p, c->nReducedRows);
        auto rreg = fetch(c, c->rrowRegion.p, c->nReducedRows);
        auto com = fetch(c, c->COM.p, R * 3);
        auto permRow = fetch(c, c->permRow.p, nA);
        auto permSys = fetch(c, c->permSys.p, nP + nT);
        std::vector<int32_t> invSys((size_t)(nP + nT));
        for (int64_t i = 0; i < nP + nT; ++i) invSys[(size_t)permSys[(size_t)i]] = (int32_t)i;
        for (int which = 0; which < 2; ++which) {
            std::vector<int64_t> ptr((size_t)nA + 1, 0);
            std::vector<int32_t> col;
            std::vector<double> val;
            std::vector<std::pair<int32_t, double>> ent;
            for (int64_t r = 0; r < nA; ++r) {
                ptr[(size_t)r] = (int64_t)val.size();
                const int row = permRow[(size_t)r];
                ent.clear();
                for (int p = sp[(size_t)row]; p < sp[(size_t)row + 1]; ++p) {
                    const int32_t rc = invSys[(size_t)sc[(size_t)p]];
                    const bool isP = rc < nP;
                    if ((which == 0) == isP) ent.push_back({isP ? rc : (int32_t)(rc - nP), sv[(size_t)p]});
                }
                std::sort(ent.begin(), ent.end());
                for (auto& e : ent) { col.push_back(e.first); val.push_back(e.second); }
            }
            ptr[(size_t)nA] = (int64_t)val.size();
            writeMarketSparse(pre + (which == 0 ? "Mat_G.mtx" : "Mat_Dt.mtx"), nA, which == 0 ? nP : nT, ptr, col, val);
        }
        for (int which = 0; which < 2; ++which) {
            std::vector<std::map<int32_t, double>> rowsM((size_t)R * PS_RD);
            for (int64_t rr = 0; rr < c->nReducedRows; ++rr) {
                int i, j, k, a;
                unpackFace(rface[(size_t)rr], i, j, k, a);
                const int reg = rreg[(size_t)rr];
                double o[3], C[PS_RD];
                faceOffset(&com[(size_t)reg * 3], c->dx, make_int3(c->gOff[0], c->gOff[1], c->gOff[2]), a, i, j, k, o);
                basisRow(o[0], o[1], o[2], a, C);
                const int64_t row = nA + rr;
                for (int p = sp[(size_t)row]; p < sp[(size_t)row + 1]; ++p) {
                    const int32_t rc = invSys[(size_t)sc[(size_t)p]];
                    const bool isP = rc < nP;
                    if ((which == 0) != isP) continue;
                    const int32_t cc = isP ? rc : (int32_t)(rc - nP);
                    for (int n = 0; n < PS_RD; ++n) rowsM[(size_t)reg * PS_RD + n][cc] += sv[(size_t)p] * C[n];
                }
            }
            std::vector<int64_t> ptr((size_t)R * PS_RD + 1, 0);
            std::vector<int32_t> col;
            std::vector<double> val;
            for (size_t r = 0; r < rowsM.size(); ++r) {
                ptr[r] = (int64_t)val.size();
                for (auto& kv : rowsM[r]) { col.push_back(kv.first); val.push_back(kv.second); }
            }
            ptr[rowsM.size()] = (int64_t)val.size();
            writeMarketSparse(pre + (which == 0 ? "Mat_JG.mtx" : "Mat_JDt.mtx"), R * PS_RD, which == 0 ? nP : nT, ptr, col, val);
        }
        auto refRows = [&](const double* dptr) {
            auto v = fetch(c, dptr, nA);
            std::vector<double> o((size_t)nA);
            for (int64_t i = 0; i < nA; ++i) o[(size_t)i] = v[(size_t)permRow[(size_t)i]];
            return o;
        };
        auto refSys = [&](const double* dptr, int64_t off, int64_t n) {
            auto v = fetch(c, dptr, nP + nT);
            std::vector<double> o((size_t)n);
            for (int64_t i = 0; i < n; ++i) o[(size_t)i] = v[(size_t)permSys[(size_t)(off + i)]];
            return o;
        };
        auto diagOut = [&](const char* name, const std::vector<double>& v) {
            const int64_t n = (int64_t)v.size();
            std::vector<int64_t> ptr((size_t)n + 1);
            std::vector<int32_t> col((size_t)n);
            for (int64_t i = 0; i <= n; ++i) ptr[(size_t)i] = i;
            for (int64_t i = 0; i < n; ++i) col[(size_t)i] = (int32_t)i;
            writeMarketSparse(pre + name, n, n, ptr, col, v);
        };
        diagOut("Mat_McInv.mtx", refRows(c->McInv.p));
        diagOut("Mat_uInv.mtx", refSys(c->uInv.p, nP, nT));
        if (c->P.exportComponentMatrices) { diagOut("Mat_Mc.mtx", refRows(c->Mc.p)); diagOut("Mat_u.mtx", refSys(c->uDiag.p, nP, nT)); }
        auto blocksWrite = [&](const char* name, const std::vector<double>& v) {
            std::vector<int64_t> ptr((size_t)R * PS_RD + 1);
            std::vector<int32_t> col((size_t)R * PS_RD * PS_RD);
            for (int64_t r = 0; r <= R * PS_RD; ++r) ptr[(size_t)r] = r * PS_RD;
            for (int64_t r = 0; r < R; ++r)
                for (int m = 0; m < PS_RD; ++m)
                    for (int n = 0; n < PS_RD; ++n) col[(size_t)((r * PS_RD + m) * PS_RD + n)] = (int32_t)(r * PS_RD + n);
            writeMarketSparse(pre + name, R * PS_RD, R * PS_RD, ptr, col, v);
        };
        auto blockOut = [&](const char* name, const double* dptr) { blocksWrite(name, fetch(c, dptr, R * PS_RD * PS_RD)); };
        blockOut("Mat_Mr.mtx", c->Mr.p);
        blockOut("Mat_JDtuDJ.mtx", c->Kv.p);
        blockOut("Mat_Inv_Mr_plus_2JDtuDJ.mtx", c->Binv.p);
        {
            auto mr = fetch(c, c->Mr.p, R * PS_RD * PS_RD), kv = fetch(c, c->Kv.p, R * PS_RD * PS_RD);
            std::vector<double> bsum(mr.size());
            for (size_t i = 0; i < mr.size(); ++i) bsum[i] = mr[i] * c->invDt + 2. * kv[i];
            blocksWrite("Mat_Mr_plus_2JDtuDJ.mtx", bsum);
        }
        {
            const std::vector<int64_t> p0(1, 0);
            writeMarketSparse(pre + "Mat_MrInv.mtx", 0, 0, p0, {}, {});
        }
        writeMarketVector(pre + "Vec_activeRHS.mtx", refRows(c->rhsA.p));
        writeMarketVector(pre + "Vec_reducedRHS.mtx", fetch(c, c->rhsR.p, R * PS_RD));
        writeMarketVector(pre + "Vec_pressureRHS.mtx", refSys(c->rhsPT.p, 0, nP));
        writeMarketVector(pre + "Vec_stressRHS.mtx", refSys(c->rhsPT.p, nP, nT));
        writeMarketVector(pre + "Vec_b.mtx", refSys(c->b.p, 0, nP + nT));
        if (c->isSolved) writeMarketVector(pre + "solutionVector.mtx", refSys(c->x.p, 0, nP + nT));
        return PS_SUCCESS;
    })
}

int32_t ps_export_matrices(ps_context* c, const char* prefix) {
    if (!c || !prefix) return PS_FAILED;
    PS_TRY(c, {
        if (!c->isSetup) throw Error("not set up");
// ... 27 lines not shown
```

polystokes_amd/csrc/ps_context.hpp:

```cpp
#pragma once
#include <map>
#include <memory>

#include "ps_common.hpp"

namespace ps {

struct DevCSR {
    int64_t rows = 0, cols = 0, nnz = 0;
    DevBuf<int32_t> ptr;
    DevBuf<int32_t> col;
    DevBuf<double> val;
    DevBuf<int8_t> code;
    bool packed = false;
    DevBuf<uint16_t> col16;
    DevBuf<int8_t> code4;
    DevBuf<double> val4;
    DevBuf<int32_t> winBase;
    DevBuf<int4> chunkInfo;
    DevBuf<uint8_t> len8;
    DevBuf<int32_t> chunkRep;
    int nChunks = 0;
    int64_t uniqueLen = 0;
    bool col16ok = false;
    int nv = 2;
    int64_t streamLen = 0;
    DevBuf<uint16_t> ecol;
    DevBuf<int8_t> ecode;
    DevBuf<int4> echunk;
    bool ellok = false;
    int64_t ellCols = 0, ellCodes = 0;
    int64_t ellUniqueCols = 0;
};

struct CGScalars {
    double rsold, pAp, alpha, beta, rr, xx, rz, rre;
    int iter;
    int done;
    int maxit;
    int pend;
    double tol2;
    int pendIter;
    int vecNT;
    double rsold2[2];
    double rrFloor, xxFix;
};

struct ArrayInfo {
    const void* dptr;
    int64_t count;
    int elem;
    const int32_t* perm = nullptr;
    int64_t permOffset = 0;
    bool host = false;
};

enum Counter : int {
    CTR_CHANGED = 0,
    CTR_ANY_FIX = 1,
    CTR_SCAN_TOTAL = 8,
    CTR_IL_PROBE = 10,
    CTR_CODE_FAIL = 20,
    CTR_COL16_FAIL_S = 22,
    CTR_COL16_FAIL_ST = 23,
    CTR_CHUNK_MAX = 25,
    CTR_DICT_OVERFLOW = 26,
    CTR_NOT_DYADIC = 40,
    CTR_HALO_UNMARKED = 41,
    CTR_ACTIVE_TOTAL = 48,
    CTR_ELL_TOO_LONG = 55,
    CTR_ELL_COLS = 56,
    CTR_ELL_CODES = 57,
    CTR_COUNT = 64
};
static_assert(CTR_ANY_FIX == CTR_CHANGED + 1, "constructCenterReducedIndices fetches the two flags together");
static_assert(CTR_IL_PROBE == CTR_SCAN_TOTAL + 2, "interleavedIndexAssignEx fetches the total and the two probes together");
static_assert(CTR_ELL_TOO_LONG == CTR_ACTIVE_TOTAL + 7 && CTR_ELL_COLS == CTR_ELL_TOO_LONG + 1 && CTR_ELL_CODES == CTR_ELL_COLS + 1,
              "seven totals, then buildEll's three values: each group is one fetch");

struct FillList {
    int32_t* p[21]; int64_t n[21];
    int count = 0;
    void add(int32_t* ptr, int64_t len) { p[count] = ptr; n[count] = len; ++count; }
};

struct FieldTable {
    static constexpr int MAX = 23;
    const float* src[MAX]; float* dst[MAX];
    int32_t fast[MAX], mid[MAX], slow[MAX];
    int count = 0;
    void add(const float* s, float* d_, int3 d, bool srcZFastest) {
        src[count] = s; dst[count] = d_;
        fast[count] = srcZFastest ? d.z : d.x; mid[count] = d.y; slow[count] = srcZFastest ? d.x : d.z;
        ++count;
    }
    int64_t entries(int q) const { return (int64_t)fast[q] * mid[q] * slow[q]; }
};
void launchFieldsCopy(const FieldTable& T, hipStream_t s);
void launchFieldsSwapXZ(const FieldTable& T, hipStream_t s);
enum ScanWord { SCAN_BAD = 0, SCAN_DIFFERS = 1, SCAN_FIRST = 2, SCAN_WORDS = 3 };
enum ScanBad { SCAN_BAD_NONE = 0, SCAN_BAD_NON_FINITE = 1, SCAN_BAD_NON_FINITE_OR_NEGATIVE = 2 };
void launchFieldScan(const float* f, int64_t n, int bad, uint32_t* out, hipStream_t s);

struct CellField;
struct FaceDensity;

}

struct ps_context {
    ps::DeferredFrees deferred;
    ps_context() { ps::MemState& M = ps::memState(); std::lock_guard<std::mutex> lk(M.m); M.lists.push_back(&deferred); ++M.contexts; }
    ~ps_context() {
        { ps::MemState& M = ps::memState(); std::lock_guard<std::mutex> lk(M.m); --M.contexts; for (size_t q = 0; q < M.lists.size(); ++q) if (M.lists[q] == &deferred) { M.lists.erase(M.lists.begin() + (long)q); break; } }
        ps::releaseDeferred(deferred);
    }
    ps_context(const ps_context&) = delete;
    ps_context& operator=(const ps_context&) = delete;
    void drainDeferred(bool streamIsIdle) {
        if (ps::threadedRanks()) return;
        if (!streamIsIdle && (!stream || hipStreamQuery(stream) != hipSuccess)) { (void)hipGetLastError(); return; }
        ps::releaseDeferred(deferred);
        ps::releaseDeferred(ps::orphanFrees());
    }
    int device = 0;
    hipStream_t stream = nullptr;
    std::string err;

    ps_params P{};
    ps::Grid g{0, 0, 0, 0};
    double dx = 0, invDx = 0, dt = 0, invDt = 0, rho = 0;
    double valScale = 0;
    bool forceFp64Values = false;
    bool haveInputWeights = false;
    bool viscUniform = false;
    float viscUniformValue = 0.f;
    double rhoScalar = 0, densMin = 0, densMax = 0;
    bool densField = false;
    int32_t densFieldHost = 0;
    bool uploaded = false, isSetup = false, isSolved = false;
    std::string uploadDensity(const float* field);
    hipEvent_t fieldEv[2] = {nullptr, nullptr};
    ps::DevBuf<uint32_t> fieldScan;
    uint32_t* pinnedScan = nullptr;
    ps::DevBuf<float> fieldScratch;
    void uploadCheck(const ps_params* p, const ps_fields_in* in) const;
    static const char* missingField(const ps_fields_in* in);
    void uploadReset(const ps_params* p, const ps_fields_in* in);
    void ingestHost(const ps_fields_in* in);
    void ingestDevice(const ps_fields_in* in, int layout, hipStream_t caller);
    void uploadTail();
    std::string checkDeviceField(const void* ptr, int64_t count, const char* name) const;
    static const char* layoutRefusal(int layout);
    std::string refuseFieldsIn(const ps_fields_in* in, int layout) const;
    void waitForCaller(hipStream_t caller);
    void releaseToCaller(hipStream_t caller);
    void moveFields(const ps::FieldTable& T, int layout) { if (layout == 0) ps::launchFieldsCopy(T, stream); else ps::launchFieldsSwapXZ(T, stream); }
    const uint32_t* scanField(const float* f, int64_t n, int bad);
    void upload(const ps_params* p, const ps_fields_in* in, int layout, hipStream_t caller);
    std::string uploadDensityDevice(const float* field, int layout, hipStream_t caller);
    void downloadDevice(const ps_fields_out* out, int layout, hipStream_t caller);
    void downloadSolutionDevice(const ps_solution_out* out, int layout, hipStream_t caller);
    double sigmaSet = 0, sigmaUsed = 0;
    ps::DevBuf<float> kappaRaw, kappaC;
    ps::DevBuf<int32_t> stReduced;
    void applySurfaceTension();
    ps::DevBuf<float> surfSigma, surfPressure;
    ps::DevBuf<double> surfQ;
    bool surfSigmaField = false, surfPressureField = false;
    int32_t surfFieldsUsed = 0;
    bool dropSurfaceFields();
    std::string uploadSurfaceFields(const ps_surface_fields* f, bool device, int layout, hipStream_t caller);
    int32_t solidBoundarySet = PS_SOLID_NO_SLIP, solidBoundaryUsed = PS_SOLID_NO_SLIP;
    ps::DevBuf<int32_t> slipEdges;
    ps_rheology rheoSet{PS_RHEOLOGY_NEWTONIAN, 0, 1., 0., 1e-3, 1e-3, 1e6};
    int32_t rheoModelUsed = PS_RHEOLOGY_NEWTONIAN;
    ps::DevBuf<float> rheoMu, rheoRate;
    bool rheoFromOut = false, rheoCarry = false;
    int rheoPass = 0;
    std::vector<int32_t> rheoIters;
    void computeRheology();
    int stepWithPasses(ps_stats* stats);
    ps::CellField viscSource() const;
    ps::FaceDensity densSource() const;

    ps::DevBuf<float> surface, collision, viscosity, density, vel[3], cvel[3];
    ps::DevBuf<double> densFace[3];
    ps::DevBuf<float> velOut[3], valid[3];

    ps::DevBuf<float> liquidW[7], fluidW[7];
    ps::DevBuf<int32_t> labels[7], activeIdx[7], reducedIdx[7];
    ps::DevBuf<int32_t> faceRow[3];
    ps::DevBuf<int32_t> sysIdx[7];
    ps::DevBuf<int32_t> sysIdxT[3];
    int ilPlaneMajor = 0;
    ps::DevBuf<int32_t> permSys, permRow;
    int ilBlocks = 0;
    std::vector<int32_t> blockStartSys, blockStartRow;
    ps::DevBuf<int32_t> cellScratch[3];
    ps::DevBuf<int32_t> scanBlock;
    ps::DevBuf<int32_t> counters;

    int64_t nCenter = 0, nFace[3] = {0, 0, 0}, nEdge[3] = {0, 0, 0};
    int64_t nActiveVs = 0, nReducedVs = 0, nPressures = 0, nStresses = 0, nSystem = 0, nTotalDOFs = 0;
    int64_t regionCount = 0;
    int64_t nReducedRows = 0;
    int64_t nRows = 0;

    ps::DevBuf<int32_t> bbox;
    std::vector<int32_t> hbbox;
    ps::DevBuf<double> COM, cfit, Mr, Kv, Binv, rhsR, regionScratch;
    struct FaceBoxItems {
        ps::DevBuf<int32_t> region, axis, start, regionPtr;
        int64_t count = 0;
    };
    FaceBoxItems fbItems;
    ps::DevBuf<unsigned long long> tileSig; ps::DevBuf<int32_t> tileUnique, tileRep, repList;
    FaceBoxItems repItems;
    int64_t tileReps = 0;
    void buildTileClasses();
    ps::DevBuf<int32_t> sbItemRegion, sbItemStart, sbItemCount, sbItemLong;
    std::vector<int32_t> skinCutsHost;
    std::vector<int32_t> sbRegionItemPtrHost;
    int64_t sbItems = 0;
    int64_t maxRegionRows = 0;
    ps::DevBuf<double> partials;

    ps::DevBuf<uint32_t> rrowFace;
    ps::DevBuf<int32_t> rrowRegion;
    ps::DevBuf<int32_t> regionRowPtr;
    ps::DevBuf<int32_t> rchunkRegion, rchunkStart, rchunkEnd, regionChunkPtr;
    int64_t nRChunks = 0;
    bool bboxValid = false;

    ps::DevCSR S, St;
    ps::DevBuf<double> McInv, rhsA, uInv, rhsPT, Mc, uDiag, oldVs;
    ps::DevBuf<uint8_t> uCode, mcCode;
    ps::DevBuf<double> uDict, mcDict;
    bool uCoded = false, mcCoded = false;
    int32_t valuesCodedHost = 0, columns16Host = 0;
    int32_t diagFlagsHost = 0;
    int32_t fusedStepHost = 0;
    static constexpr int LAUNCH_WALK_FIELDS = 8;
    int32_t launchWalkHost[5 * LAUNCH_WALK_FIELDS] = {};
    bool walkRecord = false;
    int32_t streamRunsHost[4] = {0, 0, 0, 0};
    int32_t rowPerLaneHost[2] = {0, 0};
    void buildDiagonalCodes();
    ps::DevBuf<ps::diag_t> dinvF;
    ps::DevBuf<double> b, x, r, pvec, Ap, dinv, ts, vreg, wreg, recovered, tmp1, tmp2, tmp3, tmp4, tmp5;
    ps::DevBuf<double> chebPartials, chebPartials2;
    double chebLmax = 8.4;
    bool chebInner32Req = false;
    bool chebInner32 = false;
    int32_t chebInner32Host = 0;
    ps::DevBuf<double> guess;
    int32_t warmMode = 0;
    ps::DevBuf<float> warmStore;
    bool warmHave = false;
    int warmTag[3] = {0, 0, 0};
    double warmTagDx = 0;
    ps::DevBuf<double> warmX0;
    bool warmX0Valid = false;
    int32_t warmUsedHost = 0;
    int32_t solvePrecisionSet = PS_PRECISION_FP64, solvePrecisionUsedHost = 0;
    ps::DevBuf<float> d32, p32, r32, ts32, Ap32;
    std::vector<int32_t> passIters;
    double trueResidualHost = 0;
    void dropMixedBuffers() { d32.free(); p32.free(); r32.free(); ts32.free(); Ap32.free(); }
    int32_t extrapSet = 0, extrapUsedHost = 0;
    ps::DevBuf<int8_t> extrapLayer[3];
    ps::DevBuf<int32_t> extrapCounts;
    void extrapolateVelocity(int layers);
    void dropExtrapolationBuffers() { for (auto& b : extrapLayer) b.free(); extrapCounts.free(); }
    int64_t solutionGridCount(int q) const { return g.count(q < 4 ? 0 : q); }
    void scatterSolution(float* dst, int q0, int nq);
    void carryWarmStart();
    bool gatherWarmStart();
    void dropWarmStart();
    ps::DevBuf<double> dotPartials, dotPartials2, dotPartials3, dotPartialsR;
    ps::DevBuf<double> fusedPart;
    ps::DevBuf<ps::CGScalars> scal;

    bool slabEnabled = false;
    int gOff[3] = {0, 0, 0};
    ps_slab slab{};
    ps_brick brick{};
    int64_t ownLo = 0, ownHi = 0;
    ps::DevBuf<int32_t> regionOwned;
    ps::DevBuf<int32_t> blockMap;
    int blockMapOwned = -1, blockMapFor = 0;
    static constexpr int NLINK = 6;
    struct CutList { ps::DevBuf<int32_t> idx; int64_t n = 0; uint64_t hash = 0; };
    struct Cut {
        CutList own, halo;
        ps::DevBuf<double> send, recv;
        std::vector<int32_t> hostOwn;
        const CutList& list(bool ownKind) const { return ownKind ? own : halo; }
    };
    Cut cut[NLINK][2];
    ps::DevBuf<double> redbuf;
    void ensureBuffers(int l, size_t doubles) { for (Cut& k : cut[l]) k.send.alloc(doubles); for (Cut& k : cut[l]) k.recv.alloc(doubles); }
    static void linkAxes(int l, int& a, int& b) { a = l < 3 ? l : (l == 5 ? 1 : 0); b = l < 3 ? -1 : (l == 3 ? 1 : 2); }
    int axisStride(int a) const { return a == 0 ? 1 : (a == 1 ? brick.dims[0] : brick.dims[0] * brick.dims[1]); }
    bool linked(int l, int side) const { int a, b; linkAxes(l, a, b); const int32_t* has = side ? brick.hasUpper : brick.hasLower; return has[a] && (b < 0 || has[b]); }
    int nbr(int l, int side) const { int a, b; linkAxes(l, a, b); return linked(l, side) ? brick.rank + (side ? 1 : -1) * (axisStride(a) + (b >= 0 ? axisStride(b) : 0)) : -1; }
    int64_t exchangeEntries() const { int64_t n = 0; for (const auto& l : cut) for (const Cut& k : l) n += k.own.n + k.halo.n; return n; }
    ps::DevBuf<int32_t> distList[5];
    int nDistList[5] = {0, 0, 0, 0, 0};
    bool distListsOk = false;
    hipStream_t commStream = nullptr;
    hipEvent_t distEv[8] = {nullptr, nullptr, nullptr, nullptr, nullptr, nullptr, nullptr, nullptr};
    double distStats[8] = {0, 0, 0, 0, 0, 0, 0, 0};
    ps::DevBuf<int32_t> labelFlags;
    ps::DevBuf<int32_t> fixDof, fixSrc;
    ps::DevBuf<const double*> fixBufs;
    int64_t nFix = 0;
    ps::DevBuf<unsigned char> scrMark;
    int64_t deviceShareRows = 0;
    ps::DevBuf<unsigned char> xsegTab[2];
    int nXseg[2] = {0, 0}, xsegBlocks[2] = {0, 0};
    bool haloForward = false;
    int64_t haloLabelChanges = 0;
    void* rcclComm = nullptr;
    void* hostComm = nullptr;
    ps::DevBuf<ps::CGScalars> benchScal;
    ps::DevBuf<double> benchOnes, benchZeros;
    bool ownsStream = true;
    ps::DevBuf<float> ownedFace[3];
    ps::Own own() const {
        ps::Own o;
        o.enabled = slabEnabled ? 1 : 0;
        for (int a = 0; a < 3; ++a) { o.lo[a] = brick.lo[a]; o.hi[a] = brick.hi[a]; o.hasUpper[a] = brick.hasUpper[a]; }
        return o;
    }
    void buildHaloLists();

    ps_interrupt_fn interruptCb = nullptr;
    void* interruptUser = nullptr;
    bool interrupted = false;

    int solveIterations = -1;
    double solveError = -1;
    int usedBiCGStab = 0;
    ps_stats lastStats{};

    std::map<std::string, ps::ArrayInfo> arrays;
    std::map<std::string, std::vector<char>> hostArrays;

    void upload(const ps_params* p, const ps_fields_in* in);
    void buildIntegrationWeightsAlt();
    void classifyCells();
    void constructReducedRegions();
    void constructOnlyActiveRegions();
    void classifyFaces();
    void classifyEdges();
    void constructCenterReducedIndices(int part);
    void constructFacesReducedIndices();
    void constructEdgesReducedIndices();
    void constructActiveIndices();
    void buildValidFaces();
    void computeRegionBoxes();
    void computeCenterOfMasses();
    void computeLeastSquaresFits();
    void computeReducedMassMatrices();
    void computeReducedViscosityMatricesInteriorOnly();
    void assembleReducedBlocks();
    void constructMatrixBlocks();
    void buildCol16(ps::DevCSR& M, ps::Counter failSlot, const std::vector<int32_t>& cuts, const uint8_t* rowCode, int codeRows);
    void buildEll(ps::DevCSR& M);
    void buildStreams(bool share);
    bool shareRuns = true;
    ps::DevBuf<int2> scrChunkRows; ps::DevBuf<int32_t> scrSlice, scrStart4, scrVals, scrKeep, scrRemap, scrEllCol, scrEllCode, scrEllW; ps::DevBuf<unsigned long long> scrHash, scrKeys, scrUniq;
    void ensureValues(ps::DevCSR& M);
    void buildVal4(ps::DevCSR& M);
    std::vector<int32_t> regionRowPtrHost;
    std::vector<int32_t> hostTab[20];
    void assembleSystemPressureStressFactored();
    void constructPreconditioner();
    int solve();
    void estimateLambdaMax();
    void applyPreconditionerDevice(const double* r, double* z, double* scratch);
    int chebyshevApply(const double* rvec, double* zA, double* zB, double* rzPartial, const ps::CGScalars* sc, bool firstDone = false, double** zOut = nullptr);
    double chebTheta() const;
    int ntLevel() const;
    int solveEigenCG();
    void constructGuessVectors();
    void buildExplicitA(std::vector<int64_t>& ptr, std::vector<int32_t>& col, std::vector<double>& val);
    void recoverVelocityFromPressureStress();
    void applySolutionToVelocity();
    void applyOperator(const double* x, double* y, double* dotPartialsOut);

    int setup(ps_stats* stats);
    void setupPhase(int phase);
    std::shared_ptr<void> setupState;
    int setupPhaseDone = -1;
    int solveStage(ps_stats* stats);
    void fillDimData(ps_stats* st) const;
    void registerArrays();

    int32_t orderedIndexAssign(int s, int mode, ps::DevBuf<int32_t>& out, int counterSlot = -1);
    int64_t interleavedIndexAssign(int ngroups, const int* samples, const int* weights, int32_t* const* outs);
    int64_t interleavedIndexAssignEx(int ngroups, const int* samples, const int* weights, int32_t* const* outs, bool ownFilter,
                                     int64_t* ownedRange);
    void buildInternalNumbering();
    int64_t exclusiveScanI32(int32_t* data, int64_t n, int counterSlot = -1);
    int32_t readCounter(ps::Counter idx);
    void fetchCounters(ps::Counter idx, int n, int32_t* out);
    int32_t* pinnedCounters = nullptr;
    void zeroChangeFlags();
    void fillI32(const ps::FillList& F, int32_t v);
};

void ps_bench_launch(ps_context* c, const std::string& kernel, const double* x, double* y);
int ps_dist_step_single(ps_context* c, ps_stats* stats);
void ps_dist_release(ps_context* c);

namespace ps {
constexpr int FB_CHUNK = 4096;
constexpr int PS_SCAN_TILE = 2048;
constexpr int RC_ROWS = 1280;
constexpr int TILE_FUSED_MAX_ROWS = 32768;
}
```

polystokes_amd/csrc/ps_kernels_spmv.hpp:

```cpp
#pragma once


constexpr int BS = 256;
constexpr int VGRID = 1024;

__device__ inline double waveReduceSum(double v) {
#pragma unroll
    for (int o = 32; o > 0; o >>= 1) v += __shfl_down(v, o, 64);
    return v;
}
__device__ inline double blockReduceSum(double v) {
    __shared__ double ws[BS / 64];
    const int lane = threadIdx.x & 63, w = threadIdx.x >> 6;
    v = waveReduceSum(v);
    if (lane == 0) ws[w] = v;
    __syncthreads();
    double s = 0.;
    if (threadIdx.x == 0) {
#pragma unroll
        for (int i = 0; i < BS / 64; ++i) s += ws[i];
    }
    __syncthreads();
    return s;
}
// ... 394 lines not shown
                  bufRsrc(cheb.zprev, (MODE == 2 && cheb.zprev) ? (size_t)rows * 8 : 0),
                  fusedBufs<double>(fr, rows, MODE == 3, fr.yOut != nullptr, fr.cz != nullptr)};
}
struct StRow { double e0; DiagRow u; ChebRow c; FusedRow f; };
template <int MODE, bool NT, int CAUX>
__device__ __forceinline__ StRow stRowLoads(const StBufs& B, const FusedR& fr, bool coded, unsigned row, unsigned srow) {
    StRow L{bufLoadF64epi<NT>(B.e0, row * 8u), DiagRow{0, 0.}, ChebRow{0., 0., 0.}, FusedRow{0., 0., 1.f}};
    if (MODE != 1) L.u = rowDiagLoad<CAUX, NT ? PS_EPI_AUX : 0>(coded, B.uc, B.e1, row, srow);
    if (MODE == 2) L.c = chebLoads<double>(B.cr, B.ci, B.cd, row);
    if (MODE == 3) L.f = fusedLoads<NT>(fr, B.f, row, fr.cz != nullptr);
    return L;
}
template <int MODE, bool NT>
__device__ __forceinline__ void stRowFinish(const StBufs& B, const ChebArgs& cheb, const FusedR& fr, const double* dict, bool coded, double alpha, unsigned row, bool live,
                                            const StRow& L, double s, double& dacc, double& dacc2) {
    if (MODE == 1) { bufStoreF64nt<NT>(B.out, row * 8u, -s + L.e0); return; }
    const double y = stRowY(s, rowDiagValue(coded, dict, L.u), L.e0);
    if (MODE == 0) { dacc += L.e0 * y; bufStoreF64nt<NT>(B.out, row * 8u, y); }
    else if (MODE == 2) bufStoreF64nt<NT>(B.out, row * 8u, chebRowFinish<double>(cheb, L.c, y, L.e0, dacc));
    else fusedRowFinish<NT, double>(fr, B.f, row, live, true, fr.yOut != nullptr, fr.cz != nullptr, alpha, y, L.f, dacc, dacc2);
}

struct Chunk { int q0, q1, row0, rows, src; };
__host__ __device__ inline Chunk decodeChunk(int4 v) { return Chunk{v.x, v.x + (v.y & 0xffff), v.z, (int)((unsigned)v.y >> 16), v.w}; }
#define PS_INLINE_LAMBDA __attribute__((always_inline))
template <int NV, bool F64, bool SNT, bool BNT, int ML, class Loads, class Row>
__device__ __forceinline__ bool pipeLoop(const uint16_t* __restrict__ col16, const int8_t* __restrict__ code4, const double* __restrict__ val4, int streamLen,
                                         const int32_t* __restrict__ winBase, const int4* __restrict__ chunkInfo, const uint8_t* __restrict__ len8, double scale,
                                         __amdgpu_buffer_rsrc_t rX, int rows, int nChunks, int xcdAware, const Loads& loads, const Row& finish) {
    constexpr int PL = BS * NV;
    __shared__ double prod[4 * PL];
    __shared__ __align__(16) int wtot[BS / 64];
    static_assert(BS == 256, "four waves per block");
    const __amdgpu_buffer_rsrc_t rCol = bufRsrc(col16, (size_t)streamLen * 2), rCode = bufRsrc(code4, F64 ? 0 : (size_t)streamLen), rLen = bufRsrc(len8, (size_t)rows);
    const ChunkWalk W(xcdAware);
    int it = 0;
    int chunk = W.at(0);
    if (chunk >= nChunks) return false;
    Chunk pr = decodeChunk(chunkInfo[chunk]);
    Stream4<NV, F64> cur, nxt;
    loadStream4<NV, F64, SNT>(rCol, rCode, val4, pr.q0, pr.q1, cur);
    int myBase = winBase[chunk * 16 + (threadIdx.x & 15)], nBase = 0;
    int nchunk = W.at(1);
    Chunk npr{0, 0, 0, 0, 0};
    if (nchunk < nChunks) npr = decodeChunk(chunkInfo[nchunk]);
    while (true) {
        const bool live = (int)threadIdx.x < pr.rows;
        const unsigned row = live ? (unsigned)pr.row0 + threadIdx.x : ROW_NONE, srow = live ? (unsigned)pr.src + threadIdx.x : ROW_NONE;
        const int len = (int)__builtin_amdgcn_raw_buffer_load_b8(rLen, (int)srow, 0, BNT ? PS_EPI_AUX : 0);
        const auto L = loads(row, srow);
        double xv[4 * NV];
#pragma unroll
        for (int w = 0; w < NV; ++w) {
            if (w > 0 && pr.q0 + 4 * w * BS >= pr.q1) break;
#pragma unroll
            for (int j = 0; j < 4; ++j) xv[4 * w + j] = bufGatherF64(rX, streamCol(cur.c[w], j, myBase) * 8u);
        }
        Vals4<F64 ? NV : 0> cv;
        if constexpr (F64) loadVals4<NV, SNT>(val4, pr.q0, pr.q1, cv);
        const bool hasNext = nchunk < nChunks;
        if (hasNext) {
            loadStream4<NV, F64, SNT>(rCol, rCode, val4, npr.q0, npr.q1, nxt);
            nBase = winBase[nchunk * 16 + (threadIdx.x & 15)];
        }
        const int nn = W.at(it + 2);
        Chunk nnpr{0, 0, 0, 0, 0};
        if (nn < nChunks) nnpr = decodeChunk(chunkInfo[nn]);
#pragma unroll
        for (int w = 0; w < NV; ++w) {
            if (w > 0 && pr.q0 + 4 * w * BS >= pr.q1) break;
#pragma unroll
            for (int j = 0; j < 4; ++j) prod[j * PL + threadIdx.x + w * BS] = prodVal<F64>(cur, cv, w, j, scale) * xv[4 * w + j];
        }
        const int incl = waveInclusiveScan(len);
        if ((threadIdx.x & 63) == 63) wtot[threadIdx.x >> 6] = incl;
        __syncthreads();
        {
            const int4 wt = *reinterpret_cast<const int4*>(wtot);
            const int wv = threadIdx.x >> 6;
            const int ea = incl - len + (wv > 0 ? wt.x : 0) + (wv > 1 ? wt.y : 0) + (wv > 2 ? wt.z : 0);
            finish(row, live, L, rowSum<ML, PL>(prod, ea, len));
        }
        __syncthreads();
        if (!hasNext) break;
        chunk = nchunk; pr = npr; cur = nxt; myBase = nBase;
        nchunk = nn; npr = nnpr;
        ++it;
    }
    return true;
}
template <int MODE, int NV, bool F64, int POL>
__global__ void __launch_bounds__(BS) k_spmv_S_pipe(const uint16_t* __restrict__ col16, const int8_t* __restrict__ code4, const double* __restrict__ val4, int streamLen,
                                                    const int32_t* __restrict__ winBase, const int4* __restrict__ chunkInfo,
                                                    const uint8_t* __restrict__ len8, double scale, const double* __restrict__ x, int cols, int rows,
                                                    int nA, double dt, const double* __restrict__ McInv, double* __restrict__ out,
                                                    const int* __restrict__ done, int nChunks, int xcdAware,
                                                    const uint8_t* __restrict__ mcCode, const double* __restrict__ mcDict, double* __restrict__ stPart) {
    if (done && *done) return;
    constexpr bool NT = (POL & 1) != 0, SNT = (POL & 2) != 0;
    constexpr bool BNT = NT && SNT;
    __shared__ double dict[MODE == 0 ? 256 : 1];
    const bool coded = mcCode != nullptr;
    if (MODE == 0 && coded) RowDiag<true>::fill(dict, mcDict);
    const __amdgpu_buffer_rsrc_t rX = bufRsrc(x, (size_t)cols * 8), rMc = bufRsrc(McInv, (size_t)nA * 8), rMcc = bufRsrc(mcCode, coded ? (size_t)nA : 0),
                                 rOut = bufRsrc(out, (size_t)rows * 8);
    double stAcc = 0.;
    const bool any = pipeLoop<NV, F64, SNT, BNT, 8>(col16, code4, val4, streamLen, winBase, chunkInfo, len8, scale, rX, rows, nChunks, xcdAware,
        [&](unsigned row, unsigned srow) PS_INLINE_LAMBDA { return MODE == 0 ? rowDiagLoad<BNT ? PS_EPI_AUX : 0, 0>(coded, rMcc, rMc, row, srow) : DiagRow{0, 0.}; },
        [&](unsigned row, bool, const DiagRow& m, double s) PS_INLINE_LAMBDA {
            sRowFinish<MODE, NT, double>(rOut, row, nA, dt, MODE == 0 ? rowDiagValue(coded, dict, m) : 1., s, stAcc);
        });
    if (!any) { if (MODE == 0 && stPart && threadIdx.x == 0) stPart[blockIdx.x] = 0.; return; }
    if (MODE == 0 && stPart) {
        const double bs = blockReduceSum(stAcc);
        if (threadIdx.x == 0) stPart[blockIdx.x] = bs;
    }
}
template <int MODE, int NV, bool F64, int POL>
__global__ void __launch_bounds__(BS) k_spmv_St_pipe(const uint16_t* __restrict__ col16, const int8_t* __restrict__ code4, const double* __restrict__ val4, int streamLen,
                                                     const int32_t* __restrict__ winBase, const int4* __restrict__ chunkInfo,
                                                     const uint8_t* __restrict__ len8, double scale, const double* __restrict__ t, int cols, int rows,
                                                     const double* __restrict__ uInv, const double* __restrict__ xin, const double* __restrict__ add,
                                                     double* __restrict__ out, double* __restrict__ partial, const int* __restrict__ done,
                                                     int nChunks, int xcdAware, ChebArgs cheb,
                                                     const uint8_t* __restrict__ uCode, const double* __restrict__ uDict, FusedR fr) {
    if (done && *done) return;
    constexpr bool NT = (POL & 1) != 0, SNT = (POL & 2) != 0;
    constexpr bool BNT = NT && SNT;
    __shared__ double dict[MODE != 1 ? 256 : 1];
    const bool coded = uCode != nullptr;
    if (MODE != 1 && coded) RowDiag<true>::fill(dict, uDict);
    double alpha = 0.;
    if (MODE == 3 && !fusedPrologue(fr, fr.red != nullptr, alpha)) return;
    const __amdgpu_buffer_rsrc_t rT = bufRsrc(t, (size_t)cols * 8);
    const StBufs B = stBufs<MODE>(rows, uInv, xin, add, out, cheb, uCode, coded, fr);
    double dacc = 0., dacc2 = 0.;
    const bool any = pipeLoop<NV, F64, SNT, BNT, 6>(col16, code4, val4, streamLen, winBase, chunkInfo, len8, scale, rT, rows, nChunks, xcdAware,
        [&](unsigned row, unsigned srow) PS_INLINE_LAMBDA { return stRowLoads<MODE, NT, BNT ? PS_EPI_AUX : 0>(B, fr, coded, row, srow); },
        [&](unsigned row, bool live, const StRow& L, double s) PS_INLINE_LAMBDA { stRowFinish<MODE, NT>(B, cheb, fr, dict, coded, alpha, row, live, L, s, dacc, dacc2); });
    if (!any) {
        if ((MODE == 0 || MODE == 2) && threadIdx.x == 0) partial[blockIdx.x] = 0.;
        if (MODE == 3 && threadIdx.x == 0) { fr.rPart[blockIdx.x] = 0.; fr.rPart[gridDim.x + blockIdx.x] = 0.; }
        return;
    }
    if (MODE == 0 || MODE == 2) {
        const double bs = blockReduceSum(dacc);
        if (threadIdx.x == 0) partial[blockIdx.x] = bs;
    }
    if (MODE == 3) fusedPartials(fr, dacc, dacc2, fr.cz != nullptr, (int)gridDim.x);
}


typedef unsigned int u32x3 __attribute__((ext_vector_type(3)));
struct EllUnit { int W, colByte, codeByte, row0, rows; };
__device__ inline EllUnit ellUnit(int4 ci, int wv) {
    const unsigned ws = (unsigned)ci.w >> 12;
    int pre = 0, preC = 0;
#pragma unroll
    for (int u = 0; u < 3; ++u) {
        const int w = (int)((ws >> (4 * u)) & 15u);
        if (u < wv) { pre += w; preC += w > 4 ? 8 : (w > 0 ? 4 : 0); }
    }
    EllUnit e;
    e.W = (int)((ws >> (4 * wv)) & 15u);
    e.colByte = ci.x * 2 + 128 * pre;
    e.codeByte = ci.y + 64 * preC;
    e.row0 = ci.z + 64 * wv;
    e.rows = min(64, max(0, (ci.w & 0xfff) - 64 * wv));
    if (e.rows == 0) e.W = 0;
    return e;
}
struct EllRegs { unsigned c0, c1, c2, c3, v0, v1; };
template <bool NT>
__device__ inline EllRegs ellLoad(__amdgpu_buffer_rsrc_t rCol, __amdgpu_buffer_rsrc_t rCode, const EllUnit& e, unsigned lane) {
    constexpr int AUX = NT ? PS_STREAM_AUX : 0;
    const int cb = e.colByte + (int)lane * 2 * e.W;
    EllRegs r{0u, 0u, 0u, 0u, 0u, 0u};
    if (e.W == 8) {
        const u32x4 q = __builtin_amdgcn_raw_buffer_load_b128(rCol, cb, 0, AUX);
        const u32x2 v = __builtin_amdgcn_raw_buffer_load_b64(rCode, e.codeByte + (int)lane * 8, 0, AUX);
        r = EllRegs{q.x, q.y, q.z, q.w, v.x, v.y};
    } else if (e.W == 6) {
        const u32x3 q = __builtin_amdgcn_raw_buffer_load_b96(rCol, cb, 0, AUX);
        const u32x2 v = __builtin_amdgcn_raw_buffer_load_b64(rCode, e.codeByte + (int)lane * 8, 0, AUX);
        r = EllRegs{q.x, q.y, q.z, 0u, v.x, v.y};
    } else if (e.W == 4) {
        const u32x2 q = __builtin_amdgcn_raw_buffer_load_b64(rCol, cb, 0, AUX);
        const unsigned v = __builtin_amdgcn_raw_buffer_load_b32(rCode, e.codeByte + (int)lane * 4, 0, AUX);
        r = EllRegs{q.x, q.y, 0u, 0u, v, 0u};
    } else if (e.W == 2) {
        const unsigned q = __builtin_amdgcn_raw_buffer_load_b32(rCol, cb, 0, AUX);
        const unsigned v = __builtin_amdgcn_raw_buffer_load_b32(rCode, e.codeByte + (int)lane * 4, 0, AUX);
        r = EllRegs{q, 0u, 0u, 0u, v, 0u};
    }
    return r;
}
template <int K> __device__ inline unsigned ellColWord(const EllRegs& r) { return K < 2 ? r.c0 : (K < 4 ? r.c1 : (K < 6 ? r.c2 : r.c3)); }
struct EllX { double x0, x1, x2, x3, x4, x5, x6, x7; };
template <int W, class T = double>
__device__ inline EllX ellGather(const EllRegs& r, int myBase, __amdgpu_buffer_rsrc_t rX) {
    const unsigned cw[4] = {r.c0, r.c1, r.c2, r.c3};
    double xv[8] = {0., 0., 0., 0., 0., 0., 0., 0.};
#pragma unroll
    for (int k = 0; k < W; ++k) {
        const unsigned raw = (cw[k >> 1] >> (16 * (k & 1))) & 0xffffu;
        const unsigned col = (unsigned)__shfl(myBase, (int)(raw >> 12), 16) + (raw & 4095u);
        xv[k] = VecIO<T>::gather(rX, col);
    }
    return EllX{xv[0], xv[1], xv[2], xv[3], xv[4], xv[5], xv[6], xv[7]};
}
template <class T = double>
__device__ inline EllX ellGatherW(int W, const EllRegs& r, int myBase, __amdgpu_buffer_rsrc_t rX) {
    if (W == 8) return ellGather<8, T>(r, myBase, rX);
    if (W == 6) return ellGather<6, T>(r, myBase, rX);
    if (W == 4) return ellGather<4, T>(r, myBase, rX);
    if (W == 2) return ellGather<2, T>(r, myBase, rX);
    return EllX{0., 0., 0., 0., 0., 0., 0., 0.};
}
template <int W>
__device__ inline double ellSum(const EllRegs& r, const EllX& X, double scale) {
    const unsigned vw[2] = {r.v0, r.v1};
    const double xv[8] = {X.x0, X.x1, X.x2, X.x3, X.x4, X.x5, X.x6, X.x7};
    double s = 0.;
#pragma unroll
    for (int k = 0; k < W; ++k) s += streamVal(vw[k >> 2], k & 3, scale) * xv[k];
    return s;
}
__device__ inline double ellSumW(int W, const EllRegs& r, const EllX& X, double scale) {
    if (W == 8) return ellSum<8>(r, X, scale);
    if (W == 6) return ellSum<6>(r, X, scale);
    if (W == 4) return ellSum<4>(r, X, scale);
    if (W == 2) return ellSum<2>(r, X, scale);
    return 0.;
}
template <bool SNT, bool LIST, class Loads, class Row>
__device__ __forceinline__ void ellLoop(__amdgpu_buffer_rsrc_t rCol, __amdgpu_buffer_rsrc_t rCode, __amdgpu_buffer_rsrc_t rX, const int32_t* __restrict__ winBase,
                                        const int4* __restrict__ echunk, double scale, int nChunks, int xcdAware, const int32_t* __restrict__ list,
                                        const Loads& loads, const Row& finish) {
    const ChunkWalk Wk(xcdAware);
    const unsigned lane = threadIdx.x & 63;
    const int wv = __builtin_amdgcn_readfirstlane((int)(threadIdx.x >> 6));
    int it = 0;
    int chunk = Wk.at(0);
    if (chunk >= nChunks) return;
    const int id0 = LIST ? list[chunk] : chunk;
    EllUnit cu = ellUnit(echunk[id0], wv);
    EllRegs cur = ellLoad<SNT>(rCol, rCode, cu, lane), nxt{0u, 0u, 0u, 0u, 0u, 0u};
    int myBase = winBase[id0 * 16 + (lane & 15)], nBase = 0;
    int nchunk = Wk.at(1), nid = 0;
    int4 nci = make_int4(0, 0, 0, 0);
    if (nchunk < nChunks) { nid = LIST ? list[nchunk] : nchunk; nci = echunk[nid]; }
    while (true) {
        const bool live = (int)lane < cu.rows;
        const unsigned row = live ? (unsigned)cu.row0 + lane : ROW_NONE;
        const auto L = loads(row);
        const EllX X = ellGatherW(cu.W, cur, myBase, rX);
        const bool hasNext = nchunk < nChunks;
        EllUnit nu{0, 0, 0, 0, 0};
        if (hasNext) {
            nu = ellUnit(nci, wv);
            nxt = ellLoad<SNT>(rCol, rCode, nu, lane);
            nBase = winBase[nid * 16 + (lane & 15)];
        }
        const int nn = Wk.at(it + 2);
        int nnid = 0;
        int4 nnci = make_int4(0, 0, 0, 0);
        if (nn < nChunks) { nnid = LIST ? list[nn] : nn; nnci = echunk[nnid]; }
        finish(row, live, L, ellSumW(cu.W, cur, X, scale));
        if (!hasNext) break;
        chunk = nchunk; cu = nu; cur = nxt; myBase = nBase;
        nchunk = nn; nci = nnci; nid = nnid;
        ++it;
    }
}
template <int MODE, int POL, bool LIST>
__global__ void __launch_bounds__(BS) k_spmv_S_ell(const uint16_t* __restrict__ ecol, const int8_t* __restrict__ ecode, unsigned colBytes, unsigned codeBytes,
                                                   const int32_t* __restrict__ winBase, const int4* __restrict__ echunk, double scale,
                                                   const double* __restrict__ x, int cols, int rows, int nA, double dt, const double* __restrict__ McInv,
                                                   double* __restrict__ out, const int* __restrict__ done, int nChunks, int xcdAware,
                                                   const uint8_t* __restrict__ mcCode, const double* __restrict__ mcDict, double* __restrict__ stPart,
                                                   const int32_t* __restrict__ list) {
    if (done && *done) return;
    constexpr bool NT = (POL & 1) != 0, SNT = (POL & 2) != 0;
    __shared__ double dict[MODE == 0 ? 256 : 1];
    const bool coded = mcCode != nullptr;
    if (MODE == 0 && coded) RowDiag<true>::fill(dict, mcDict);
    __syncthreads();
    const __amdgpu_buffer_rsrc_t rCol = bufRsrc(ecol, colBytes), rCode = bufRsrc(ecode, codeBytes), rX = bufRsrc(x, (size_t)cols * 8),
                                 rMc = bufRsrc(McInv, (size_t)nA * 8), rMcc = bufRsrc(mcCode, coded ? (size_t)nA : 0), rOut = bufRsrc(out, (size_t)rows * 8);
    double stAcc = 0.;
    ellLoop<SNT, LIST>(rCol, rCode, rX, winBase, echunk, scale, nChunks, xcdAware, list,
        [&](unsigned row) PS_INLINE_LAMBDA { return MODE == 0 ? rowDiagLoad<NT ? PS_EPI_AUX : 0, 0>(coded, rMcc, rMc, row, row) : DiagRow{0, 0.}; },
        [&](unsigned row, bool, const DiagRow& m, double s) PS_INLINE_LAMBDA {
            sRowFinish<MODE, NT, double>(rOut, row, nA, dt, MODE == 0 ? rowDiagValue(coded, dict, m) : 1., s, stAcc);
        });
    if (MODE == 0 && stPart) {
        const double bs = blockReduceSum(stAcc);
        if (threadIdx.x == 0) stPart[blockIdx.x] = bs;
    }
}
template <int MODE, int POL, int FX, bool LIST>
__global__ void __launch_bounds__(BS) k_spmv_St_ell(const uint16_t* __restrict__ ecol, const int8_t* __restrict__ ecode, unsigned colBytes, unsigned codeBytes,
                                                    const int32_t* __restrict__ winBase, const int4* __restrict__ echunk, double scale,
                                                    const double* __restrict__ t, int cols, int rows, const double* __restrict__ uInv,
                                                    const double* __restrict__ xin, const double* __restrict__ add, double* __restrict__ out,
                                                    double* __restrict__ partial, const int* __restrict__ done, int nChunks, int xcdAware, ChebArgs cheb,
                                                    const uint8_t* __restrict__ uCode, const double* __restrict__ uDict, FusedR fr, const int32_t* __restrict__ list) {
    if (done && *done) return;
    constexpr bool NT = (POL & 1) != 0, SNT = (POL & 2) != 0;
    static_assert(FX == 0 || MODE == 3, "FX: MODE 3 only");
    if (FX & 1) { fr.cz = nullptr; fr.dinvC = nullptr; uInv = nullptr; }
    if (FX & 2) { fr.yOut = nullptr; fr.rStride = 0; fr.red = nullptr; fr.ownLo = 0; fr.ownHi = rows; }
    if (FX & 4) { fr.yOut = nullptr; fr.ownLo = 0; fr.ownHi = rows; }
    const bool coded = (FX & 1) ? true : uCode != nullptr;
    __shared__ double dict[MODE != 1 ? 256 : 1];
    if (MODE != 1 && coded) RowDiag<true>::fill(dict, uDict);
    double alpha = 0.;
    if (MODE == 3 && !fusedPrologue(fr, fr.red != nullptr, alpha)) return;
    __syncthreads();
    const __amdgpu_buffer_rsrc_t rCol = bufRsrc(ecol, colBytes), rCode = bufRsrc(ecode, codeBytes), rT = bufRsrc(t, (size_t)cols * 8);
    const StBufs B = stBufs<MODE>(rows, uInv, xin, add, out, cheb, uCode, coded, fr);
    double dacc = 0., dacc2 = 0.;
    ellLoop<SNT, LIST>(rCol, rCode, rT, winBase, echunk, scale, nChunks, xcdAware, list,
        [&](unsigned row) PS_INLINE_LAMBDA { return stRowLoads<MODE, NT, NT ? PS_EPI_AUX : 0>(B, fr, coded, row, row); },
        [&](unsigned row, bool live, const StRow& L, double s) PS_INLINE_LAMBDA { stRowFinish<MODE, NT>(B, cheb, fr, dict, coded, alpha, row, live, L, s, dacc, dacc2); });
    if (MODE == 0 || MODE == 2) {
        const double bs = blockReduceSum(dacc);
        if (threadIdx.x == 0) partial[blockIdx.x] = bs;
    }
    if (MODE == 3) fusedPartials(fr, dacc, dacc2, fr.cz != nullptr, fr.rStride > 0 ? fr.rStride : (int)gridDim.x);
}

__host__ __device__ inline int pairWalkEnd(int nChunks) { return ((((nChunks + 1) >> 1) + 255) >> 8) << 5; }
__host__ __device__ inline int pairWalkChunk(int q, int xcd, int half, int nChunks) {
    const int pair = ((((q >> 5) << 3) + xcd) << 5) + (q & 31);
    const int ch = 2 * pair + half;
    return (pair < ((nChunks + 1) >> 1) && ch < nChunks) ? ch : -1;
}
template <bool LIST> struct PairWalk {
    int nChunks, xcd, half, per, qEnd;
    const int32_t* list;
    __device__ PairWalk(int n, int half_, const int32_t* list_)
        : nChunks(n), xcd(blockIdx.x & 7), half(half_), per(gridDim.x >> 3), qEnd(pairWalkEnd(n)), list(list_) {}
    __device__ int first() const { return blockIdx.x >> 3; }
    __device__ int at(int q) const {
        const int ch = q < qEnd ? pairWalkChunk(q, xcd, half, nChunks) : -1;
        return (LIST && ch >= 0) ? list[ch] : ch;
    }
};
template <bool SNT, bool LIST, class TX, class Loads, class Row>
__device__ __forceinline__ void ell2Loop(__amdgpu_buffer_rsrc_t rCol, __amdgpu_buffer_rsrc_t rCode, __amdgpu_buffer_rsrc_t rX, const int32_t* __restrict__ winBase,
                                         const int4* __restrict__ echunk, double scale, int nChunks, const int32_t* __restrict__ list, const Loads& loads, const Row& finish) {
    const unsigned lane = threadIdx.x & 63;
    const int wv = __builtin_amdgcn_readfirstlane((int)(threadIdx.x >> 6));
    const int u0 = 2 * (wv & 1);
    const PairWalk<LIST> W(nChunks, wv >> 1, list);
    int q = W.first();
    int chunk = W.at(q);
    int4 ci = make_int4(0, 0, 0, 0);
    int myBase = 0;
    if (chunk >= 0) { ci = echunk[chunk]; myBase = winBase[chunk * 16 + (lane & 15)]; }
    while (q < W.qEnd) {
        const int qn = q + W.per;
        const int nchunk = W.at(qn);
        int4 nci = make_int4(0, 0, 0, 0);
        int nBase = 0;
        if (chunk >= 0) {
            const EllUnit ua = ellUnit(ci, u0), ub = ellUnit(ci, u0 + 1);
            const EllRegs sa = ellLoad<SNT>(rCol, rCode, ua, lane), sb = ellLoad<SNT>(rCol, rCode, ub, lane);
            if (nchunk >= 0) { nci = echunk[nchunk]; nBase = winBase[nchunk * 16 + (lane & 15)]; }
            const bool liveA = (int)lane < ua.rows, liveB = (int)lane < ub.rows;
            const unsigned rowA = liveA ? (unsigned)ua.row0 + lane : ROW_NONE, rowB = liveB ? (unsigned)ub.row0 + lane : ROW_NONE;
            const auto LA = loads(rowA);
            const auto LB = loads(rowB);
            const EllX XA = ellGatherW<TX>(ua.W, sa, myBase, rX);
            const EllX XB = ellGatherW<TX>(ub.W, sb, myBase, rX);
            const double a = ellSumW(ua.W, sa, XA, scale), b = ellSumW(ub.W, sb, XB, scale);
            finish(rowA, liveA, LA, a);
            finish(rowB, liveB, LB, b);
        } else if (nchunk >= 0) { nci = echunk[nchunk]; nBase = winBase[nchunk * 16 + (lane & 15)]; }
        q = qn; chunk = nchunk; ci = nci; myBase = nBase;
    }
}
template <int POL, bool LIST, class TV, bool MC>
__device__ __forceinline__ void spmvSEll2(const uint16_t* __restrict__ ecol, const int8_t* __restrict__ ecode, unsigned colBytes, unsigned codeBytes,
                                          const int32_t* __restrict__ winBase, const int4* __restrict__ echunk, double scale,
                                          const TV* __restrict__ x, int cols, int rows, int nA, double dt, TV* __restrict__ out,
                                          const int* __restrict__ done, int nChunks, const uint8_t* __restrict__ mcCode, const double* __restrict__ mcDict,
                                          double* __restrict__ stPart, const int32_t* __restrict__ list) {
    if (done && *done) return;
    constexpr bool NT = (POL & 1) != 0, SNT = (POL & 2) != 0;
    __shared__ double dict[MC ? 256 : 1];
    RowDiag<MC>::fill(dict, mcDict);
    __syncthreads();
    const __amdgpu_buffer_rsrc_t rCol = bufRsrc(ecol, colBytes), rCode = bufRsrc(ecode, codeBytes), rX = bufRsrc(x, (size_t)cols * sizeof(TV)),
                                 rMcc = bufRsrc(mcCode, MC ? (size_t)nA : (size_t)nA * 8), rOut = bufRsrc(out, (size_t)rows * sizeof(TV));
    double stAcc = 0.;
    ell2Loop<SNT, LIST, TV>(rCol, rCode, rX, winBase, echunk, scale, nChunks, list,
        [&](unsigned row) PS_INLINE_LAMBDA { return RowDiag<MC>::template load<NT ? PS_EPI_AUX : 0>(rMcc, row, row); },
        [&](unsigned row, bool, const DiagRow& m, double s) PS_INLINE_LAMBDA { sRowFinish<0, NT, TV>(rOut, row, nA, dt, RowDiag<MC>::value(dict, m), s, stAcc); });
    if (stPart) {
        const double bs = blockReduceSum(stAcc);
        if (threadIdx.x == 0) stPart[blockIdx.x] = bs;
    }
}
#define PS_S_ELL2_PARAMS const uint16_t* __restrict__ ecol, const int8_t* __restrict__ ecode, unsigned colBytes, unsigned codeBytes, \
                         const int32_t* __restrict__ winBase, const int4* __restrict__ echunk, double scale, const TV* __restrict__ x, int cols, int rows, \
                         int nA, double dt, TV* __restrict__ out, const int* __restrict__ done, int nChunks, const uint8_t* __restrict__ mcCode, \
                         const double* __restrict__ mcDict, double* __restrict__ stPart, const int32_t* __restrict__ list
#define PS_S_ELL2_ARGS ecol, ecode, colBytes, codeBytes, winBase, echunk, scale, x, cols, rows, nA, dt, out, done, nChunks, mcCode, mcDict, stPart, list
template <int POL, bool LIST, class TV = double>
__global__ void __launch_bounds__(BS) k_spmv_S_ell2(PS_S_ELL2_PARAMS) { spmvSEll2<POL, LIST, TV, true>(PS_S_ELL2_ARGS); }
template <int POL, bool LIST, class TV = double>
__global__ void __launch_bounds__(BS) k_spmv_S_ell2u(PS_S_ELL2_PARAMS) { spmvSEll2<POL, LIST, TV, false>(PS_S_ELL2_ARGS); }
#undef PS_S_ELL2_ARGS
#undef PS_S_ELL2_PARAMS

template <int POL, bool CZ, bool DIST, bool LIST, class TZ = double, bool HALO = false, bool UC = true, class TV = double, bool AP = false>
__global__ void __launch_bounds__(BS) __attribute__((amdgpu_waves_per_eu(6, 6))) k_spmv_St_ell2(const uint16_t* __restrict__ ecol, const int8_t* __restrict__ ecode, unsigned colBytes, unsigned codeBytes,
                                                     const int32_t* __restrict__ winBase, const int4* __restrict__ echunk, double scale,
                                                     const TV* __restrict__ t, int cols, int rows, const TV* __restrict__ xin,
                                                     const int* __restrict__ done, int nChunks, const uint8_t* __restrict__ uCode, const double* __restrict__ uDict, FusedR fr,
                                                     const int32_t* __restrict__ list) {
    if (done && *done) return;
    constexpr bool NT = (POL & 1) != 0, SNT = (POL & 2) != 0, PASS = !std::is_same<TV, double>::value;
    static_assert(!HALO || DIST, "halo rows exist on a rank of a decomposition only");
    static_assert(!AP || (PASS && !CZ && !DIST && !HALO), "the plain product: single-domain passes of the mixed-precision solve only");
    __shared__ double dict[UC ? 256 : 1];
    RowDiag<UC>::fill(dict, uDict);
    double alpha;
    if constexpr (AP) alpha = 0.; else if (!fusedPrologue<PASS>(fr, DIST, alpha)) return;
    __syncthreads();
    const __amdgpu_buffer_rsrc_t rCol = bufRsrc(ecol, colBytes), rCode = bufRsrc(ecode, codeBytes), rT = bufRsrc(t, (size_t)cols * sizeof(TV)),
                                 rE0 = bufRsrc(xin, (size_t)rows * sizeof(TV)), rUc = bufRsrc(uCode, UC ? (size_t)rows : (size_t)rows * 8);
    const FusedBufs B = fusedBufs<TZ, TV>(fr, rows, true, HALO, CZ);
    struct Loaded { double e; DiagRow u; FusedRow f; };
    double dacc = 0., dacc2 = 0.;
    ell2Loop<SNT, LIST, TV>(rCol, rCode, rT, winBase, echunk, scale, nChunks, list,
        [&](unsigned row) PS_INLINE_LAMBDA {
            return Loaded{VecIO<TV>::template loadEpi<NT>(rE0, row), RowDiag<UC>::template load<NT ? (UC ? PS_UC_AUX : PS_EPI_AUX) : 0>(rUc, row, row),
                          AP ? FusedRow{0., 0., 1.f} : fusedLoads<NT, TV>(fr, B, row, CZ)};
        },
        [&](unsigned row, bool live, const Loaded& L, double s) PS_INLINE_LAMBDA {
            const double y = stRowY(s, RowDiag<UC>::value(dict, L.u), L.e);
            if constexpr (AP) { dacc += L.e * y; VecIO<TV>::template store<NT>(B.r, row, y); }
            else fusedRowFinish<NT, TZ, TV>(fr, B, row, live, HALO, HALO, CZ, alpha, y, L.f, dacc, dacc2);
        });
    if constexpr (AP) {
        const double bs = blockReduceSum(dacc);
        if (threadIdx.x == 0) fr.rPart[blockIdx.x] = bs;
    } else
    fusedPartials(fr, dacc, dacc2, CZ, (DIST && fr.rStride > 0) ? fr.rStride : (int)gridDim.x);
}

#ifdef PS_ST2C_WAVES
#define PS_ST2C_ATTR __attribute__((amdgpu_waves_per_eu(PS_ST2C_WAVES, PS_ST2C_WAVES)))
#else
#define PS_ST2C_ATTR
#endif
template <int POL, class TV = double, bool UC = true>
__global__ void __launch_bounds__(BS) PS_ST2C_ATTR k_spmv_St_ell2c(const uint16_t* __restrict__ ecol, const int8_t* __restrict__ ecode, unsigned colBytes, unsigned codeBytes,
                                                      const int32_t* __restrict__ winBase, const int4* __restrict__ echunk, double scale,
                                                      const TV* __restrict__ t, int cols, int rows, const TV* __restrict__ xin, TV* __restrict__ out,
                                                      double* __restrict__ partial, const int* __restrict__ done, int nChunks, ChebArgs cheb,
                                                      const uint8_t* __restrict__ uCode, const double* __restrict__ uDict) {
    if (done && *done) return;
    constexpr bool NT = (POL & 1) != 0, SNT = (POL & 2) != 0;
    __shared__ double dict[UC ? 256 : 1];
    RowDiag<UC>::fill(dict, uDict);
    __syncthreads();
    const __amdgpu_buffer_rsrc_t rCol = bufRsrc(ecol, colBytes), rCode = bufRsrc(ecode, codeBytes), rT = bufRsrc(t, (size_t)cols * sizeof(TV)),
                                 rE0 = bufRsrc(xin, (size_t)rows * sizeof(TV)), rUc = bufRsrc(uCode, UC ? (size_t)rows : (size_t)rows * 8), rOut = bufRsrc(out, (size_t)rows * sizeof(TV)),
                                 rCr = bufRsrc(cheb.r, (size_t)rows * 8), rCi = bufRsrc(cheb.dinv, (size_t)rows * sizeof(diag_t)),
                                 rCd = bufRsrc(cheb.zprev, cheb.zprev ? (size_t)rows * sizeof(TV) : 0);
    struct Loaded { double e; DiagRow u; ChebRow c; };
    double dacc = 0.;
    ell2Loop<SNT, false, TV>(rCol, rCode, rT, winBase, echunk, scale, nChunks, nullptr,
        [&](unsigned row) PS_INLINE_LAMBDA {
            return Loaded{VecIO<TV>::template loadEpi<NT>(rE0, row), RowDiag<UC>::template load<NT ? (UC ? PS_UC_AUX : PS_EPI_AUX) : 0>(rUc, row, row), chebLoads<TV>(rCr, rCi, rCd, row)};
        },
        [&](unsigned row, bool, const Loaded& L, double s) PS_INLINE_LAMBDA {
            VecIO<TV>::template store<NT>(rOut, row, chebRowFinish<TV>(cheb, L.c, stRowY(s, RowDiag<UC>::value(dict, L.u), L.e), L.e, dacc));
        });
    const double bs = blockReduceSum(dacc);
    if (threadIdx.x == 0) partial[blockIdx.x] = bs;
}
#undef PS_INLINE_LAMBDA
```

Before: 1042 ms/step.

## Store one shared code word for ELL units whose rows share identical value codes

During ELL construction, each 64-row unit is checked for whether all rows carry the same code bytes. Such units are marked in the packed width word and store a single 8-byte code run instead of one per lane. The SpMV loop then reads that word with a scalar load rather than a per-lane buffer load, cutting value-code traffic. It also forces 8 waves per EU on the S ELL2 kernel, which may limit registers, and adds a counting kernel used for verbose output and byte accounting.

```diff
diff --git a/polystokes_amd/__init__.py b/polystokes_amd/__init__.py
--- a/polystokes_amd/__init__.py
+++ b/polystokes_amd/__init__.py
@@ -215,7 +215,7 @@
 def _kind(name):
     if name.endswith(("Labels", "Indices", ".col", ".ptr", "Region", "Perm", ".chunkInfo", ".chunkRep", ".code")) or name.startswith("faceRow"):
         return "i"
-    if name in ("valuesCoded", "columns16", "diagonalsCoded", "fusedStep", "streamRuns", "rowPerLane", "chebInner32", "warmStartUsed", "densityField", "launchWalk",
+    if name in ("valuesCoded", "columns16", "diagonalsCoded", "fusedStep", "streamRuns", "uniformCodeUnits", "rowPerLane", "chebInner32", "warmStartUsed", "densityField", "launchWalk",
                 "surfaceTensionReducedFaces", "surfaceFields", "solidBoundary", "solidSlipEdges", "rheologyModel", "rheologyIterations",
                 "solvePrecisionUsed", "solvePassIterations",
                 "velocityExtrapolation", "extrapolationLayerX", "extrapolationLayerY", "extrapolationLayerZ", "extrapolationCounts"):
diff --git a/polystokes_amd/csrc/ps_blocks.hip b/polystokes_amd/csrc/ps_blocks.hip
--- a/polystokes_amd/csrc/ps_blocks.hip
+++ b/polystokes_amd/csrc/ps_blocks.hip
@@ -554,26 +554,66 @@
 }
 __device__ inline int ellCodeWidth(int W) { return W > 4 ? 8 : (W > 0 ? 4 : 0); }
 constexpr int32_t ELL_NULL_BASE = 0x1ffff000;
+__device__ inline int ellCodeRun(int W, bool uniform) { return uniform ? 8 : 64 * ellCodeWidth(W); }
 __global__ void __launch_bounds__(BS) k_ell_plan(const int4* __restrict__ chunkInfo, const uint8_t* __restrict__ len8, const int32_t* __restrict__ chunkRep,
+                                                 const int8_t* __restrict__ code4, int mark,
                                                  int32_t* __restrict__ colLen, int32_t* __restrict__ codeLen, int32_t* __restrict__ wpack, int32_t* __restrict__ fail) {
-    __shared__ int wmax[BS / 64];
+    __shared__ int wmax[BS / 64], wuni[BS / 64];
+    __shared__ int lastE0;
     const int chunk = blockIdx.x;
     const int4 ci = chunkInfo[chunk];
     const int rows = (int)((unsigned)ci.y >> 16);
-    int len = (int)threadIdx.x < rows ? (int)len8[ci.z + threadIdx.x] : 0;
-    for (int o = 32; o > 0; o >>= 1) len = max(len, __shfl_down(len, o, 64));
-    if ((threadIdx.x & 63) == 0) wmax[threadIdx.x >> 6] = len;
+    const bool own = chunkRep[chunk] == chunk;
+    const int lenRow = (int)len8[ci.z + min((int)threadIdx.x, rows - 1)];
+    const int mine = (int)threadIdx.x < rows ? lenRow : 0;
+    int len = mine;
+    for (int o = 32; o > 0; o >>= 1) len = max(len, __shfl_xor(len, o, 64));
+    const int W = (len + 1) & ~1;
+    bool uni = false;
+    if (mark && own) {
+        int total;
+        const int e0 = blockExclusiveScan(mine, &total);
+        if ((int)threadIdx.x == rows - 1) lastE0 = e0;
+        __syncthreads();
+        if (W > 0 && W <= 8) {
+            const int eb = ci.x + ((int)threadIdx.x < rows ? e0 : lastE0);
+            unsigned lo = 0u, hi = 0u;
+            for (int k = 0; k < min(lenRow, 8); ++k) {
+                const unsigned b = (unsigned)(uint8_t)code4[eb + k];
+                if (k < 4) lo |= b << (8 * k); else hi |= b << (8 * (k - 4));
+            }
+            uni = __all(lo == (unsigned)__builtin_amdgcn_readfirstlane((int)lo) && hi == (unsigned)__builtin_amdgcn_readfirstlane((int)hi)) != 0;
+        }
+    }
+    if ((threadIdx.x & 63) == 0) { wmax[threadIdx.x >> 6] = len; wuni[threadIdx.x >> 6] = uni ? 1 : 0; }
     __syncthreads();
     if (threadIdx.x == 0) {
         int cl = 0, vl = 0, wp = 0;
         for (int u = 0; u < BS / 64; ++u) {
-            const int W = (wmax[u] + 1) & ~1;
-            if (W > 8) *fail = 1;
-            cl += 64 * W; vl += 64 * ellCodeWidth(W); wp |= (W & 15) << (4 * u);
-        }
-        const bool own = chunkRep[chunk] == chunk;
+            const int Wu = (wmax[u] + 1) & ~1;
+            if (Wu > 8) *fail = 1;
+            cl += 64 * Wu; vl += ellCodeRun(Wu, wuni[u] != 0); wp |= ((Wu & 15) << (4 * u)) | (wuni[u] << (16 + u));
+        }
         colLen[chunk] = own ? cl : 0; codeLen[chunk] = own ? vl : 0; wpack[chunk] = wp;
     }
+}
+__global__ void __launch_bounds__(BS) k_ell_count(const int4* __restrict__ echunk, const uint8_t* __restrict__ len8, int nChunks, int32_t* __restrict__ ctr) {
+    const int lane = threadIdx.x & 63;
+    int units = 0, marked = 0, ent = 0;
+    for (int chunk = blockIdx.x * (BS / 64) + (int)(threadIdx.x >> 6); chunk < nChunks; chunk += gridDim.x * (BS / 64)) {
+        const int4 ci = echunk[chunk];
+        const unsigned ws = (unsigned)ci.w >> 12;
+        const int rows = ci.w & 0xfff;
+        for (int u = 0; u < BS / 64; ++u) {
+            if (((ws >> (4 * u)) & 15u) == 0u || 64 * u >= rows) continue;
+            ++units;
+            if (!((ws >> (16 + u)) & 1u)) continue;
+            ++marked;
+            if (64 * u + lane < rows) ent += (int)len8[ci.z + 64 * u + lane];
+        }
+    }
+    for (int o = 32; o > 0; o >>= 1) ent += __shfl_xor(ent, o, 64);
+    if (lane == 0) { atomicAdd(ctr, units); atomicAdd(ctr + 1, marked); atomicAdd(ctr + 2, ent); }
 }
 __global__ void __launch_bounds__(BS) k_ell_fill(const int4* __restrict__ chunkInfo, const uint8_t* __restrict__ len8, const int32_t* __restrict__ chunkRep,
                                                  const uint16_t* __restrict__ col16, const int8_t* __restrict__ code4, const int32_t* __restrict__ colBegin,
@@ -586,8 +626,8 @@
     if (nullOk && threadIdx.x == 0) winBase[chunk * 16 + 15] = ELL_NULL_BASE;
     const int4 ci = chunkInfo[chunk];
     const int rows = (int)((unsigned)ci.y >> 16);
-    const int wp = wpack[chunk];
-    if (threadIdx.x == 0) echunk[chunk] = make_int4(colBegin[rep], codeBegin[rep], ci.z, rows | (wp << 12));
+    const int wp = (wpack[chunk] & 0xffff) | (wpack[rep] & 0xf0000);
+    if (threadIdx.x == 0) echunk[chunk] = make_int4(colBegin[rep], codeBegin[rep], ci.z, (int)((unsigned)rows | ((unsigned)wp << 12)));
     if (rep != chunk) return;
     const int len = (int)len8[ci.z + min((int)threadIdx.x, rows - 1)];
     int total;
@@ -600,20 +640,23 @@
     const int u = threadIdx.x >> 6, lane = threadIdx.x & 63;
     const int W = (wp >> (4 * u)) & 15, CW = ellCodeWidth(W);
     if (W == 0 || u * 64 >= rows) return;
+    const bool uni = ((wp >> (16 + u)) & 1) != 0;
     int pre = 0, preC = 0;
-    for (int v = 0; v < u; ++v) { const int w = (wp >> (4 * v)) & 15; pre += w; preC += ellCodeWidth(w); }
+    for (int v = 0; v < u; ++v) { const int w = (wp >> (4 * v)) & 15; pre += w; preC += ellCodeRun(w, ((wp >> (16 + v)) & 1) != 0); }
     uint16_t* oc = ecol + (size_t)colBegin[chunk] + (size_t)64 * pre + (size_t)lane * W;
-    int8_t* ov = ecode + (size_t)codeBegin[chunk] + (size_t)64 * preC + (size_t)lane * CW;
+    int8_t* ov = ecode + (size_t)codeBegin[chunk] + (size_t)preC + (uni ? (size_t)0 : (size_t)lane * CW);
     uint16_t lastc = 0;
     for (int k = 0; k < W; ++k) {
         if (k < len) lastc = col16[eb + k];
         oc[k] = (k < len || !nullOk) ? lastc : (uint16_t)0xf000;
     }
-    for (int k = 0; k < CW; ++k) ov[k] = k < len ? code4[eb + k] : (int8_t)0;
+    if (uni && lane != 0) return;
+    for (int k = 0; k < (uni ? 8 : CW); ++k) ov[k] = k < len ? code4[eb + k] : (int8_t)0;
 }
 }
 void ps_context::buildEll(ps::DevCSR& M) {
     M.ellok = false;
+    M.ellUnits = M.ellMarked = M.ellMarkedEntries = 0; M.ellCounted = false;
     static const bool off = envInt(PS_ENV("PS_NO_ELL"), 0) != 0 ||
                             envInt(PS_ENV("PS_PIPE_GRID"), 1) == 0;
     if (off || !M.col16ok || !M.packed || M.nChunks == 0 || (uint64_t)std::max(M.rows, M.cols) * 8 >= 0xffff8000ull) return;
@@ -622,9 +665,10 @@
     colBegin.alloc((size_t)nChunks + 1); codeBegin.alloc((size_t)nChunks + 1); wpack.alloc((size_t)nChunks);
     HIP_CHECK(hipMemsetAsync(colBegin.p + nChunks, 0, sizeof(int32_t), stream));
     HIP_CHECK(hipMemsetAsync(codeBegin.p + nChunks, 0, sizeof(int32_t), stream));
+    static const int mark = envInt(PS_ENV("PS_NO_UNIFORM_CODES"), 0) != 0 ? 0 : 1;
     HIP_CHECK(hipMemsetAsync(counters.p + CTR_ELL_TOO_LONG, 0, sizeof(int32_t), stream));
     hipLaunchKernelGGL(k_ell_plan, dim3((unsigned)nChunks), dim3(BS), 0, stream, (const int4*)M.chunkInfo.p, (const uint8_t*)M.len8.p, (const int32_t*)M.chunkRep.p,
-                       colBegin.p, codeBegin.p, wpack.p, counters.p + CTR_ELL_TOO_LONG);
+                       (const int8_t*)M.code4.p, mark, colBegin.p, codeBegin.p, wpack.p, counters.p + CTR_ELL_TOO_LONG);
     scanBlock.alloc((size_t)gridFor(nChunks + 1, PS_SCAN_TILE) + 16);
     (void)exclusiveScanI32(colBegin.p, nChunks + 1, CTR_ELL_COLS);
     (void)exclusiveScanI32(codeBegin.p, nChunks + 1, CTR_ELL_CODES);
@@ -639,8 +683,22 @@
                        (const uint16_t*)M.col16.p, (const int8_t*)M.code4.p, (const int32_t*)colBegin.p, (const int32_t*)codeBegin.p, (const int32_t*)wpack.p,
                        M.ecol.p, M.ecode.p, M.echunk.p, M.winBase.p);
     M.ellok = true;
-    if (PS_ENV_VERBOSE()) std::fprintf(stderr, "[polystokes] row-per-lane stream: %d chunks, %lld column slots and %lld code bytes in the distinct runs (nnz %lld)\n",
-                                           nChunks, (long long)totCol, (long long)totCode, (long long)M.nnz);
+    if (PS_ENV_VERBOSE()) {
+        ellCounts(M);
+        std::fprintf(stderr, "[polystokes] row-per-lane stream: %d chunks, %lld column slots and %lld code bytes in the distinct runs (nnz %lld), "
+                             "uniform-code units %lld of %lld\n",
+                     nChunks, (long long)totCol, (long long)totCode, (long long)M.nnz, (long long)M.ellMarked, (long long)M.ellUnits);
+    }
+}
+void ps_context::ellCounts(ps::DevCSR& M) {
+    if (M.ellCounted || !M.ellok) return;
+    HIP_CHECK(hipMemsetAsync(counters.p + CTR_ELL_UNITS, 0, 3 * sizeof(int32_t), stream));
+    hipLaunchKernelGGL(k_ell_count, dim3((unsigned)std::min(256, gridFor(M.nChunks, BS / 64))), dim3(BS), 0, stream, (const int4*)M.echunk.p, (const uint8_t*)M.len8.p,
+                       M.nChunks, counters.p + CTR_ELL_UNITS);
+    int32_t w[3];
+    fetchCounters(CTR_ELL_UNITS, 3, w);
+    M.ellUnits = w[0]; M.ellMarked = w[1]; M.ellMarkedEntries = w[2];
+    M.ellCounted = true;
 }
 namespace {
 __global__ void k_decode_values(const int8_t* __restrict__ code, double scale, int64_t n, double* __restrict__ val) {
diff --git a/polystokes_amd/csrc/ps_context.hip b/polystokes_amd/csrc/ps_context.hip
--- a/polystokes_amd/csrc/ps_context.hip
+++ b/polystokes_amd/csrc/ps_context.hip
@@ -412,6 +412,7 @@
     streamRunsHost[0] = S.col16ok ? (int32_t)S.uniqueLen : 0; streamRunsHost[1] = S.col16ok ? (int32_t)S.streamLen : 0;
     streamRunsHost[2] = St.col16ok ? (int32_t)St.uniqueLen : 0; streamRunsHost[3] = St.col16ok ? (int32_t)St.streamLen : 0;
     regHost("streamRuns", streamRunsHost, 4, 4);
+    regHost("uniformCodeUnits", uniformCodeUnitsHost, 4, 4);
     rowPerLaneHost[0] = ((S.ellok && S.packed) ? 1 : 0) | ((St.ellok && St.packed) ? 2 : 0); rowPerLaneHost[1] = ilPlaneMajor;
     regHost("rowPerLane", rowPerLaneHost, 2, 4);
     reg("sysPerm", permSys.p, nSystem, 4);
@@ -979,6 +980,12 @@
             c->ensureValues(M);
             c->arrays[name].dptr = M.val.p;
         }
+        if (c->isSetup && std::strcmp(name, "uniformCodeUnits") == 0) {
+            HIP_CHECK(hipSetDevice(c->device));
+            c->ellCounts(c->S); c->ellCounts(c->St);
+            const int32_t v[4] = {(int32_t)c->S.ellMarked, (int32_t)c->S.ellUnits, (int32_t)c->St.ellMarked, (int32_t)c->St.ellUnits};
+            std::memcpy(c->uniformCodeUnitsHost, v, sizeof(v));
+        }
         auto it = c->arrays.find(name);
         if (it == c->arrays.end()) throw Error(std::string("unknown array ") + name);
         const int64_t need = it->second.count * it->second.elem;
@@ -1063,8 +1070,10 @@
             auto ell = [&](const ps::DevCSR& M) { return c16(M) && M.packed && M.ellok && !fp64; };
             const double ptrS = c16(c->S) ? (ell(c->S) ? 0. : 1.) : 4., ptrT = c16(c->St) ? (ell(c->St) ? 0. : 1.) : 4.;
             const double dMc = (c16(c->S) && c->mcCoded) ? 1. : 8., dU = (c16(c->St) && c->uCoded) ? 1. : 8.;
-            const double bS = winS + perNnzS * entS + ptrS * (rowsS + 1) + 8. * rowsS + 8. * rowsT + dMc * (double)c->nActiveVs;
-            const double bT = winT + perNnzT * entT + ptrT * (rowsT + 1) + 8. * rowsT + 8. * rowsS + 8. * rowsT + dU * rowsT;
+            c->ellCounts(c->S); c->ellCounts(c->St);
+            auto uniS = [&](const ps::DevCSR& M) { return ell(M) ? 8. * (double)M.ellMarked - (double)M.ellMarkedEntries : 0.; };
+            const double bS = winS + uniS(c->S) + perNnzS * entS + ptrS * (rowsS + 1) + 8. * rowsS + 8. * rowsT + dMc * (double)c->nActiveVs;
+            const double bT = winT + uniS(c->St) + perNnzT * entT + ptrT * (rowsT + 1) + 8. * rowsT + 8. * rowsS + 8. * rowsT + dU * rowsT;
             const double dg = c->P.preconditioner == PS_PRE_DIAGONAL ? (double)sizeof(ps::diag_t) : 0.;
             if (kb == "spmv_S") *algorithmic_bytes = bS;
             else if (kb == "spmv_St") *algorithmic_bytes = bT;
diff --git a/polystokes_amd/csrc/ps_context.hpp b/polystokes_amd/csrc/ps_context.hpp
--- a/polystokes_amd/csrc/ps_context.hpp
+++ b/polystokes_amd/csrc/ps_context.hpp
@@ -31,6 +31,8 @@
     bool ellok = false;
     int64_t ellCols = 0, ellCodes = 0;
     int64_t ellUniqueCols = 0;
+    int64_t ellUnits = 0, ellMarked = 0, ellMarkedEntries = 0;
+    bool ellCounted = false;
 };
 
 struct CGScalars {
@@ -71,12 +73,14 @@
     CTR_ELL_TOO_LONG = 55,
     CTR_ELL_COLS = 56,
     CTR_ELL_CODES = 57,
+    CTR_ELL_UNITS = 58,
     CTR_COUNT = 64
 };
 static_assert(CTR_ANY_FIX == CTR_CHANGED + 1, "constructCenterReducedIndices fetches the two flags together");
 static_assert(CTR_IL_PROBE == CTR_SCAN_TOTAL + 2, "interleavedIndexAssignEx fetches the total and the two probes together");
 static_assert(CTR_ELL_TOO_LONG == CTR_ACTIVE_TOTAL + 7 && CTR_ELL_COLS == CTR_ELL_TOO_LONG + 1 && CTR_ELL_CODES == CTR_ELL_COLS + 1,
               "seven totals, then buildEll's three values: each group is one fetch");
+static_assert(CTR_ELL_UNITS + 3 <= CTR_COUNT, "ellCounts fetches three values");
 
 struct FillList {
     int32_t* p[21]; int64_t n[21];
@@ -244,6 +248,7 @@
     int32_t launchWalkHost[5 * LAUNCH_WALK_FIELDS] = {};
     bool walkRecord = false;
     int32_t streamRunsHost[4] = {0, 0, 0, 0};
+    int32_t uniformCodeUnitsHost[4] = {0, 0, 0, 0};
     int32_t rowPerLaneHost[2] = {0, 0};
     void buildDiagonalCodes();
     ps::DevBuf<ps::diag_t> dinvF;
@@ -371,6 +376,7 @@
     void buildStreams(bool share);
     bool shareRuns = true;
     ps::DevBuf<int2> scrChunkRows; ps::DevBuf<int32_t> scrSlice, scrStart4, scrVals, scrKeep, scrRemap, scrEllCol, scrEllCode, scrEllW; ps::DevBuf<unsigned long long> scrHash, scrKeys, scrUniq;
+    void ellCounts(ps::DevCSR& M);
     void ensureValues(ps::DevCSR& M);
     void buildVal4(ps::DevCSR& M);
     std::vector<int32_t> regionRowPtrHost;
diff --git a/polystokes_amd/csrc/ps_kernels_spmv.hpp b/polystokes_amd/csrc/ps_kernels_spmv.hpp
--- a/polystokes_amd/csrc/ps_kernels_spmv.hpp
+++ b/polystokes_amd/csrc/ps_kernels_spmv.hpp
@@ -570,46 +570,60 @@
 
 
 typedef unsigned int u32x3 __attribute__((ext_vector_type(3)));
-struct EllUnit { int W, colByte, codeByte, row0, rows; };
+struct EllUnit { int W, colByte, codeByte, row0, rows; bool uni; };
 __device__ inline EllUnit ellUnit(int4 ci, int wv) {
     const unsigned ws = (unsigned)ci.w >> 12;
     int pre = 0, preC = 0;
 #pragma unroll
     for (int u = 0; u < 3; ++u) {
         const int w = (int)((ws >> (4 * u)) & 15u);
-        if (u < wv) { pre += w; preC += w > 4 ? 8 : (w > 0 ? 4 : 0); }
+        if (u < wv) { pre += w; preC += ((ws >> (16 + u)) & 1u) ? 8 : (w > 4 ? 512 : (w > 0 ? 256 : 0)); }
     }
     EllUnit e;
     e.W = (int)((ws >> (4 * wv)) & 15u);
     e.colByte = ci.x * 2 + 128 * pre;
-    e.codeByte = ci.y + 64 * preC;
+    e.codeByte = ci.y + preC;
     e.row0 = ci.z + 64 * wv;
     e.rows = min(64, max(0, (ci.w & 0xfff) - 64 * wv));
     if (e.rows == 0) e.W = 0;
+    e.uni = ((ws >> (16 + wv)) & 1u) != 0;
     return e;
 }
 struct EllRegs { unsigned c0, c1, c2, c3, v0, v1; };
-template <bool NT>
+struct EllWord { unsigned u0, u1; };
+__device__ inline EllWord ellWord(const int8_t* __restrict__ ecode, const EllUnit& e) {
+    if (!e.uni) return EllWord{0u, 0u};
+    const unsigned* w = reinterpret_cast<const unsigned*>(ecode + e.codeByte);
+    return EllWord{w[0], w[1]};
+}
+template <int N, int AUX, bool WORD>
+__device__ inline u32x2 ellCodes(__amdgpu_buffer_rsrc_t rCode, const EllUnit& e, unsigned lane) {
+    if (WORD && e.uni) return u32x2{0u, 0u};
+    const int at = e.codeByte + ((!WORD && e.uni) ? 0 : (int)lane * (4 * N));
+    if (N == 2) return __builtin_amdgcn_raw_buffer_load_b64(rCode, at, 0, AUX);
+    return u32x2{__builtin_amdgcn_raw_buffer_load_b32(rCode, at, 0, AUX), 0u};
+}
+template <bool NT, bool WORD>
 __device__ inline EllRegs ellLoad(__amdgpu_buffer_rsrc_t rCol, __amdgpu_buffer_rsrc_t rCode, const EllUnit& e, unsigned lane) {
     constexpr int AUX = NT ? PS_STREAM_AUX : 0;
     const int cb = e.colByte + (int)lane * 2 * e.W;
     EllRegs r{0u, 0u, 0u, 0u, 0u, 0u};
     if (e.W == 8) {
         const u32x4 q = __builtin_amdgcn_raw_buffer_load_b128(rCol, cb, 0, AUX);
-        const u32x2 v = __builtin_amdgcn_raw_buffer_load_b64(rCode, e.codeByte + (int)lane * 8, 0, AUX);
+        const u32x2 v = ellCodes<2, AUX, WORD>(rCode, e, lane);
         r = EllRegs{q.x, q.y, q.z, q.w, v.x, v.y};
     } else if (e.W == 6) {
         const u32x3 q = __builtin_amdgcn_raw_buffer_load_b96(rCol, cb, 0, AUX);
-        const u32x2 v = __builtin_amdgcn_raw_buffer_load_b64(rCode, e.codeByte + (int)lane * 8, 0, AUX);
+        const u32x2 v = ellCodes<2, AUX, WORD>(rCode, e, lane);
         r = EllRegs{q.x, q.y, q.z, 0u, v.x, v.y};
     } else if (e.W == 4) {
         const u32x2 q = __builtin_amdgcn_raw_buffer_load_b64(rCol, cb, 0, AUX);
-        const unsigned v = __builtin_amdgcn_raw_buffer_load_b32(rCode, e.codeByte + (int)lane * 4, 0, AUX);
-        r = EllRegs{q.x, q.y, 0u, 0u, v, 0u};
+        const u32x2 v = ellCodes<1, AUX, WORD>(rCode, e, lane);
+        r = EllRegs{q.x, q.y, 0u, 0u, v.x, v.y};
     } else if (e.W == 2) {
         const unsigned q = __builtin_amdgcn_raw_buffer_load_b32(rCol, cb, 0, AUX);
-        const unsigned v = __builtin_amdgcn_raw_buffer_load_b32(rCode, e.codeByte + (int)lane * 4, 0, AUX);
-        r = EllRegs{q, 0u, 0u, 0u, v, 0u};
+        const u32x2 v = ellCodes<1, AUX, WORD>(rCode, e, lane);
+        r = EllRegs{q, 0u, 0u, 0u, v.x, v.y};
     }
     return r;
 }
@@ -650,6 +664,10 @@
     if (W == 4) return ellSum<4>(r, X, scale);
     if (W == 2) return ellSum<2>(r, X, scale);
     return 0.;
+}
+__device__ inline double ellSumU(const EllUnit& e, const EllRegs& r, const EllWord& k, const EllX& X, double scale) {
+    if (e.uni) return ellSumW(e.W, EllRegs{r.c0, r.c1, r.c2, r.c3, k.u0, k.u1}, X, scale);
+    return ellSumW(e.W, r, X, scale);
 }
 template <bool SNT, bool LIST, class Loads, class Row>
 __device__ __forceinline__ void ellLoop(__amdgpu_buffer_rsrc_t rCol, __amdgpu_buffer_rsrc_t rCode, __amdgpu_buffer_rsrc_t rX, const int32_t* __restrict__ winBase,
@@ -663,7 +681,7 @@
     if (chunk >= nChunks) return;
     const int id0 = LIST ? list[chunk] : chunk;
     EllUnit cu = ellUnit(echunk[id0], wv);
-    EllRegs cur = ellLoad<SNT>(rCol, rCode, cu, lane), nxt{0u, 0u, 0u, 0u, 0u, 0u};
+    EllRegs cur = ellLoad<SNT, false>(rCol, rCode, cu, lane), nxt{0u, 0u, 0u, 0u, 0u, 0u};
     int myBase = winBase[id0 * 16 + (lane & 15)], nBase = 0;
     int nchunk = Wk.at(1), nid = 0;
     int4 nci = make_int4(0, 0, 0, 0);
@@ -674,10 +692,10 @@
         const auto L = loads(row);
         const EllX X = ellGatherW(cu.W, cur, myBase, rX);
         const bool hasNext = nchunk < nChunks;
-        EllUnit nu{0, 0, 0, 0, 0};
+        EllUnit nu{0, 0, 0, 0, 0, false};
         if (hasNext) {
             nu = ellUnit(nci, wv);
-            nxt = ellLoad<SNT>(rCol, rCode, nu, lane);
+            nxt = ellLoad<SNT, false>(rCol, rCode, nu, lane);
             nBase = winBase[nid * 16 + (lane & 15)];
         }
         const int nn = Wk.at(it + 2);
@@ -767,7 +785,7 @@
     }
 };
 template <bool SNT, bool LIST, class TX, class Loads, class Row>
-__device__ __forceinline__ void ell2Loop(__amdgpu_buffer_rsrc_t rCol, __amdgpu_buffer_rsrc_t rCode, __amdgpu_buffer_rsrc_t rX, const int32_t* __restrict__ winBase,
+__device__ __forceinline__ void ell2Loop(__amdgpu_buffer_rsrc_t rCol, __amdgpu_buffer_rsrc_t rCode, const int8_t* __restrict__ ecode, __amdgpu_buffer_rsrc_t rX, const int32_t* __restrict__ winBase,
                                          const int4* __restrict__ echunk, double scale, int nChunks, const int32_t* __restrict__ list, const Loads& loads, const Row& finish) {
     const unsigned lane = threadIdx.x & 63;
     const int wv = __builtin_amdgcn_readfirstlane((int)(threadIdx.x >> 6));
@@ -785,7 +803,8 @@
         int nBase = 0;
         if (chunk >= 0) {
             const EllUnit ua = ellUnit(ci, u0), ub = ellUnit(ci, u0 + 1);
-            const EllRegs sa = ellLoad<SNT>(rCol, rCode, ua, lane), sb = ellLoad<SNT>(rCol, rCode, ub, lane);
+            const EllWord ka = ellWord(ecode, ua), kb = ellWord(ecode, ub);
+            const EllRegs sa = ellLoad<SNT, true>(rCol, rCode, ua, lane), sb = ellLoad<SNT, true>(rCol, rCode, ub, lane);
             if (nchunk >= 0) { nci = echunk[nchunk]; nBase = winBase[nchunk * 16 + (lane & 15)]; }
             const bool liveA = (int)lane < ua.rows, liveB = (int)lane < ub.rows;
             const unsigned rowA = liveA ? (unsigned)ua.row0 + lane : ROW_NONE, rowB = liveB ? (unsigned)ub.row0 + lane : ROW_NONE;
@@ -793,7 +812,7 @@
             const auto LB = loads(rowB);
             const EllX XA = ellGatherW<TX>(ua.W, sa, myBase, rX);
             const EllX XB = ellGatherW<TX>(ub.W, sb, myBase, rX);
-            const double a = ellSumW(ua.W, sa, XA, scale), b = ellSumW(ub.W, sb, XB, scale);
+            const double a = ellSumU(ua, sa, ka, XA, scale), b = ellSumU(ub, sb, kb, XB, scale);
             finish(rowA, liveA, LA, a);
             finish(rowB, liveB, LB, b);
         } else if (nchunk >= 0) { nci = echunk[nchunk]; nBase = winBase[nchunk * 16 + (lane & 15)]; }
@@ -814,7 +833,7 @@
     const __amdgpu_buffer_rsrc_t rCol = bufRsrc(ecol, colBytes), rCode = bufRsrc(ecode, codeBytes), rX = bufRsrc(x, (size_t)cols * sizeof(TV)),
                                  rMcc = bufRsrc(mcCode, MC ? (size_t)nA : (size_t)nA * 8), rOut = bufRsrc(out, (size_t)rows * sizeof(TV));
     double stAcc = 0.;
-    ell2Loop<SNT, LIST, TV>(rCol, rCode, rX, winBase, echunk, scale, nChunks, list,
+    ell2Loop<SNT, LIST, TV>(rCol, rCode, ecode, rX, winBase, echunk, scale, nChunks, list,
         [&](unsigned row) PS_INLINE_LAMBDA { return RowDiag<MC>::template load<NT ? PS_EPI_AUX : 0>(rMcc, row, row); },
         [&](unsigned row, bool, const DiagRow& m, double s) PS_INLINE_LAMBDA { sRowFinish<0, NT, TV>(rOut, row, nA, dt, RowDiag<MC>::value(dict, m), s, stAcc); });
     if (stPart) {
@@ -828,7 +847,7 @@
                          const double* __restrict__ mcDict, double* __restrict__ stPart, const int32_t* __restrict__ list
 #define PS_S_ELL2_ARGS ecol, ecode, colBytes, codeBytes, winBase, echunk, scale, x, cols, rows, nA, dt, out, done, nChunks, mcCode, mcDict, stPart, list
 template <int POL, bool LIST, class TV = double>
-__global__ void __launch_bounds__(BS) k_spmv_S_ell2(PS_S_ELL2_PARAMS) { spmvSEll2<POL, LIST, TV, true>(PS_S_ELL2_ARGS); }
+__global__ void __launch_bounds__(BS) __attribute__((amdgpu_waves_per_eu(8, 8))) k_spmv_S_ell2(PS_S_ELL2_PARAMS) { spmvSEll2<POL, LIST, TV, true>(PS_S_ELL2_ARGS); }
 template <int POL, bool LIST, class TV = double>
 __global__ void __launch_bounds__(BS) k_spmv_S_ell2u(PS_S_ELL2_PARAMS) { spmvSEll2<POL, LIST, TV, false>(PS_S_ELL2_ARGS); }
 #undef PS_S_ELL2_ARGS
@@ -854,7 +873,7 @@
     const FusedBufs B = fusedBufs<TZ, TV>(fr, rows, true, HALO, CZ);
     struct Loaded { double e; DiagRow u; FusedRow f; };
     double dacc = 0., dacc2 = 0.;
-    ell2Loop<SNT, LIST, TV>(rCol, rCode, rT, winBase, echunk, scale, nChunks, list,
+    ell2Loop<SNT, LIST, TV>(rCol, rCode, ecode, rT, winBase, echunk, scale, nChunks, list,
         [&](unsigned row) PS_INLINE_LAMBDA {
             return Loaded{VecIO<TV>::template loadEpi<NT>(rE0, row), RowDiag<UC>::template load<NT ? (UC ? PS_UC_AUX : PS_EPI_AUX) : 0>(rUc, row, row),
                           AP ? FusedRow{0., 0., 1.f} : fusedLoads<NT, TV>(fr, B, row, CZ)};
@@ -893,7 +912,7 @@
                                  rCd = bufRsrc(cheb.zprev, cheb.zprev ? (size_t)rows * sizeof(TV) : 0);
     struct Loaded { double e; DiagRow u; ChebRow c; };
     double dacc = 0.;
-    ell2Loop<SNT, false, TV>(rCol, rCode, rT, winBase, echunk, scale, nChunks, nullptr,
+    ell2Loop<SNT, false, TV>(rCol, rCode, ecode, rT, winBase, echunk, scale, nChunks, nullptr,
         [&](unsigned row) PS_INLINE_LAMBDA {
             return Loaded{VecIO<TV>::template loadEpi<NT>(rE0, row), RowDiag<UC>::template load<NT ? (UC ? PS_UC_AUX : PS_EPI_AUX) : 0>(rUc, row, row), chebLoads<TV>(rCr, rCi, rCd, row)};
         },
```

Measured after the change: 1043 ms/step (median of 3 runs). About the same (+0.0%).
